# uzh-rpg/EvDeblurNeRF

Hardware: AMD Instinct MI355X
Metric: rays/sec (4096x128 samples, 8x256 MLP) (higher is better)
Workload: dtype f16c (compensated f16: one f16 MFMA product + two block-scaled fp6 MFMA products of the operands' rounding residuals; f32 accumulate; ~2^-15 operands); 1 GPU; nerf8x256 render: 4096 rays x 128 samples per GPU, PE(10,4)+MLP+composite, ndc, viewdirs; rays_per_gpu=4096, samples=128, precision=f16c

## Files before the change

### evdeblurnerf_amd/_lib.py

```python
from __future__ import annotations

import ctypes as C
import os

_HERE = os.path.dirname(os.path.abspath(__file__))
LIB_PATH = os.environ.get("EVD_LIB_PATH") or os.path.join(_HERE, "lib", "libevdnerf.so")
MAXL = 16

PREC = {"f32": 0, "f16x3": 1, "bf16": 2, "f16": 3, "f16c": 4, "f16m": 5}
ACT = {"none": 0, "relu": 1, "sigmoid": 2, "exp": 3, "sigmoid1": 4, "softplus": 5, "tanh": 6}

_fp = C.POINTER(C.c_float)
_vp = C.c_void_p


class EvdError(RuntimeError):
    pass


class RenderCfg(C.Structure):
    _fields_ = [("H", C.c_int), ("W", C.c_int), ("focal", C.c_float),
                ("ndc", C.c_int), ("use_viewdirs", C.c_int), ("lindisp", C.c_int), ("N_samples", C.c_int),
                ("N_importance", C.c_int), ("white_bkgd", C.c_int),
                ("near", C.c_float), ("far", C.c_float), ("perturb", C.c_float),
                ("is_train", C.c_int), ("precision", C.c_int)]


class NerfDesc(C.Structure):
    _fields_ = [("D", C.c_int), ("W", C.c_int), ("multires", C.c_int), ("multires_views", C.c_int), ("skip", C.c_int),
                ("rgb_act", C.c_int), ("sigma_act", C.c_int), ("rmnear", C.c_float),
                ("pts_w", _fp * MAXL), ("pts_b", _fp * MAXL),
                ("views_w", _fp), ("views_b", _fp), ("feature_w", _fp), ("feature_b", _fp),
                ("alpha_w", _fp), ("alpha_b", _fp), ("rgb_w", _fp), ("rgb_b", _fp),
                ("output_w", _fp), ("output_b", _fp), ("output_ch", C.c_int)]


class NerfGrads(C.Structure):
    _fields_ = [("pts_w", _vp * MAXL), ("pts_b", _vp * MAXL),
                ("views_w", _vp), ("views_b", _vp), ("feature_w", _vp), ("feature_b", _vp),
                ("alpha_w", _vp), ("alpha_b", _vp), ("rgb_w", _vp), ("rgb_b", _vp), ("accumulate", C.c_int)]


class VoxelGrads(C.Structure):
    _fields_ = [("sigma_w", _vp * 2), ("color_w", _vp * 3), ("color_b", _vp * 3), ("accumulate", C.c_int)]


class AwpEmbedGrads(C.Structure):
    _fields_ = [("w", _vp * 4), ("b", _vp * 4)]


class AwpTailDesc(C.Structure):
    _fields_ = [("P", C.c_int), ("S", C.c_int), ("VF", C.c_int), ("dir_freqs", C.c_int), ("n_mot", C.c_int), ("training", C.c_int),
                ("bn_eps", C.c_float), ("bn_momentum", C.c_float)]


class VoxelGridGrads(C.Structure):
    _fields_ = [("plane", _vp * 3), ("line", _vp * 3), ("basis", _vp)]


class VoxelDesc(C.Structure):
    _fields_ = [("num_layers", C.c_int), ("hidden_dim", C.c_int), ("geo_feat_dim", C.c_int),
                ("num_layers_color", C.c_int), ("input_ch", C.c_int), ("multires", C.c_int), ("multires_views", C.c_int),
                ("app_dim", C.c_int), ("n_comp", C.c_int * 3), ("grid", C.c_int * 3), ("app_act", C.c_int),
                ("rgb_act", C.c_int), ("sigma_act", C.c_int), ("composite_feature", C.c_int),
                ("aabb", C.c_float * 6), ("rmnear", C.c_float),
                ("sigma_w", _fp * MAXL), ("color_w", _fp * MAXL), ("color_b", _fp * MAXL),
                ("plane", _fp * 3), ("line", _fp * 3), ("basis", _fp)]


class CrfDesc(C.Structure):
    _fields_ = [("map_type", C.c_int), ("gamma", C.c_float), ("extra_features", C.c_int),
                ("w", _fp * 4), ("b", _fp * 4)]


class PoseTrack(C.Structure):
    _fields_ = [("n_keys", C.c_int), ("key_t", _vp), ("key_quat", _vp), ("key_rotvec", _vp), ("trans_coef", _vp),
                ("bd_scale", C.c_float), ("recenter", C.c_int), ("recenter_inv", C.c_double * 12)]


class RigidBlurDesc(C.Structure):
    _fields_ = [(k, C.c_int) for k in ("C", "W_r", "W_v", "W_w", "D_r", "D_v", "D_w", "M", "use_origin", "n_img")] + [("rv_window", C.c_float)]


class RigidBlurParams(C.Structure):
    _fields_ = [(k, _vp) for k in ("table", "r_branch_w", "r_branch_b", "v_branch_w", "v_branch_b", "w_branch_w", "w_branch_b",
                                   "r_linear_w", "r_linear_b", "v_linear_w", "v_linear_b", "w_linear_w", "w_linear_b")]


class LpipsDesc(C.Structure):
    _fields_ = [("conv_w", _fp * 5), ("conv_b", _fp * 5), ("lin", _fp * 5), ("shift", C.c_float * 3), ("scale", C.c_float * 3)]


class RenderOut(C.Structure):
    _fields_ = [(k, _vp) for k in ("rgb", "depth", "acc", "z_vals", "weights", "rgb0", "depth0", "acc0", "z_std",
                                   "z_vals0", "weights0", "feature", "raw")] + [("feature_kind", C.c_int)]


_L, _I, _F, _S = C.c_long, C.c_int, C.c_float, C.c_size_t
SIGNATURES = {
    "evd_last_error": (C.c_char_p, []),
    "evd_version": (_I, []),
    "evd_debug_side_spin_count": (_L, []),
    "evd_compute_successor_workspace_bytes": (_S, [_L]),
    "evd_compute_successor": (_I, [_vp, _L, _L, _vp, _vp, _vp, _vp, _vp, _S, _vp]),
    "evd_event_coord_ids_workspace_bytes": (_S, [_L, _I, _I]),
    "evd_event_coord_ids": (_I, [_vp, _vp, _L, _I, _I, _vp, _vp, _vp, _vp, _vp, _S, _vp]),
    "evd_event_filter_workspace_bytes": (_S, [_L]),
    "evd_event_filter": (_I, [_vp, _vp, _vp, _L, C.c_double, C.c_double, _vp, _vp, _vp, _vp, _S, _vp]),
    "evd_event_color_map_workspace_bytes": (_S, [_L]),
    "evd_event_color_map": (_I, [_vp, _L, _I, _I, _vp, _vp, _vp, _L, _vp, _vp, _vp, _S, _vp]),
    "evd_sample_events": (_I, [_vp, _L, _I, _vp, _L, _vp, _vp, _vp, _vp, _L, _fp, _I, _vp, _vp, _vp, _vp, _vp, _vp, _vp, _vp, _vp]),
    "evd_sample_events_track": (_I, [_vp, _L, _I, _vp, _L, _vp, C.POINTER(PoseTrack), _vp, _vp, _L, _fp, _I, _vp, _vp, _vp, _vp, _vp, _vp, _vp, _vp, _vp]),
    "evd_interpolate_poses": (_I, [C.POINTER(PoseTrack), _vp, _L, _vp, _vp]),
    "evd_image_batch": (_I, [_vp, _L, _vp, _vp, _vp, _I, _I, _I, _fp, _vp, _vp, _vp, _vp, _vp, _vp, _vp, _vp, _vp]),
    "evd_rbk_warp": (_I, [_vp, _vp, _vp, _L, _I, _I, _vp, _vp, _vp]),
    "evd_rigid_blur_workspace_bytes": (_S, [C.POINTER(RigidBlurDesc), _L]),
    "evd_rigid_blur_forward": (_I, [C.POINTER(RigidBlurDesc), C.POINTER(RigidBlurParams), _vp, _vp, _vp, _L, _vp, _vp, _vp, _vp]),
    "evd_rigid_blur_backward": (_I, [C.POINTER(RigidBlurDesc), C.POINTER(RigidBlurParams), _vp, _vp, _vp, _L, _vp, _vp, _vp, _vp, _vp, _vp,
                                     _vp, _S, _vp]),
    "evd_awp_feature_integration": (_I, [_vp, _vp, _vp, _L, _I, _I, _vp, _vp]),
    "evd_awp_feature_integration_bwd": (_I, [_vp, _vp, _vp, _vp, _L, _I, _I, _vp, _vp, _vp, _vp]),
    "evd_mam_local_forward": (_I, [_vp, _vp, _L, _I, _I, _I, _vp, _vp, _vp, _vp, _vp]),
    "evd_mam_local_backward": (_I, [_vp, _vp, _vp, _vp, _vp, _vp, _vp, _vp, _L, _I, _I, _I, _vp, _vp, _I, _vp, _vp]),
    "evd_awp_tail_num_params": (_I, [_I]),
    "evd_awp_tail_param_count": (_L, [C.POINTER(AwpTailDesc)]),
    "evd_awp_tail_workspace_bytes": (_S, [C.POINTER(AwpTailDesc), _L, _I]),
    "evd_awp_tail_saved_floats": (_L, [C.POINTER(AwpTailDesc)]),
    "evd_awp_tail_forward": (_I, [C.POINTER(AwpTailDesc), C.POINTER(_vp), _vp, _vp, _vp, _vp, _vp, _L, _vp, _vp, _vp, _vp, _vp, _vp, _vp, _vp, _vp, _S, _vp]),
    "evd_awp_tail_backward": (_I, [C.POINTER(AwpTailDesc), C.POINTER(_vp), _vp, _vp, _vp, _vp, _vp, _L, _vp, _vp, _vp, _vp, _vp, _vp, _vp, _vp, _vp,
                                   _vp, _vp, _vp, _S, _vp]),
    "evd_awp_local_consumers_backward": (_I, [_vp] * 11 + [_L, _I, _I, _I, _vp, _vp, _vp, _vp, _vp, _vp]),
    "evd_awp_embed_create": (_I, [C.POINTER(_fp), C.POINTER(_fp), _I, _I, _I, C.POINTER(_vp)]),
    "evd_awp_embed_destroy": (None, [_vp]),
    "evd_awp_embed_param_count": (_L, [_vp]),
    "evd_awp_embed_load_params": (_I, [_vp, _vp, _vp]),
    "evd_awp_embed_store_bytes": (_S, [_vp, _L]),
    "evd_awp_embed_backward_workspace_bytes": (_S, []),
    "evd_awp_embed_forward": (_I, [_vp, _I, _vp, _vp, _vp, _S, _L, _vp, _vp, _S, _vp]),
    "evd_awp_embed_backward": (_I, [_vp, _I, _vp, _L, _vp, _S, C.POINTER(AwpEmbedGrads), _vp, _vp, _vp, _S, _vp]),
    "evd_probe_mfma_rate": (_I, [_I, _I, C.POINTER(C.c_double), _vp]),
    "evd_device_count": (_I, []),
    "evd_get_rays": (_I, [_I, _I, _fp, _fp, _I, _vp, _vp, _vp]),
    "evd_get_rays_pix": (_I, [_vp, _fp, _vp, _L, _I, _vp, _vp, _vp]),
    "evd_ndc_rays": (_I, [_I, _I, _F, _F, _vp, _vp, _L, _vp, _vp, _vp]),
    "evd_embed": (_I, [_vp, _L, _I, _I, _vp, _vp]),
    "evd_ray_batch": (_I, [C.POINTER(RenderCfg), _vp, _L, _vp, _vp]),
    "evd_ray_batch_bwd": (_I, [C.POINTER(RenderCfg), _vp, _vp, _L, _vp, _vp]),
    "evd_points": (_I, [_vp, _I, _vp, _L, _I, _vp, _vp]),
    "evd_points_bwd": (_I, [_vp, _vp, _L, _I, _I, _vp, _vp]),
    "evd_sample_z": (_I, [C.POINTER(RenderCfg), _vp, _I, _L, _vp, _vp, _vp]),
    "evd_sample_z_pts": (_I, [C.POINTER(RenderCfg), _vp, _I, _L, _vp, _vp, _vp, _vp]),
    "evd_ray_batch_z": (_I, [C.POINTER(RenderCfg), _vp, _L, _vp, _vp, _vp, _vp]),
    "evd_nerf_create": (_I, [C.POINTER(NerfDesc), C.POINTER(_vp)]),
    "evd_nerf_destroy": (None, [_vp]),
    "evd_nerf_param_count": (_L, [_vp]),
    "evd_nerf_param_blocks": (_I, [_vp, C.POINTER(C.c_long), _I]),
    "evd_nerf_load_params": (_I, [_vp, _vp, _vp]),
    "evd_nerf_stream_bytes": (_S, [_vp, _I]),
    "evd_nerf_mlp": (_I, [_vp, _I, _vp, _vp, _L, _I, _vp, _vp, _I, _vp]),
    "evd_nerf_train_store_bytes": (_S, [_L]),
    "evd_nerf_train_store_bytes_prec": (_S, [_I, _L]),
    "evd_nerf_mlp_train": (_I, [_vp, _I, _vp, _vp, _L, _I, _vp, _vp, _S, _vp]),
    "evd_nerf_backward_workspace_bytes": (_S, []),
    "evd_nerf_mlp_backward": (_I, [_vp, _I, _vp, _L, _I, _vp, _S, C.POINTER(NerfGrads), _vp, _vp, _I, _vp, _vp, _vp, _S, _vp]),
    "evd_voxel_param_count": (_L, [_vp]),
    "evd_voxel_param_blocks": (_I, [_vp, C.POINTER(C.c_long), _I]),
    "evd_voxel_load_params": (_I, [_vp, _vp, _vp]),
    "evd_voxel_train_store_bytes": (_S, [_vp, _L]),
    "evd_voxel_train_store_bytes_prec": (_S, [_vp, _I, _L]),
    "evd_voxel_backward_workspace_bytes": (_S, []),
    "evd_voxel_mlp_train": (_I, [_vp, _I, _vp, _vp, _I, _vp, _I, _L, _I, _vp, _vp, _vp, _S, _vp]),
    "evd_voxel_geo_feat_dim": (_I, [_vp]),
    "evd_voxel_mlp_backward": (_I, [_vp, _I, _vp, _vp, _vp, _vp, _S, _L, _I, _vp, _S, C.POINTER(VoxelGrads), _vp, _I, _vp, _vp, _I, _vp, _vp, _vp, _S, _vp]),
    "evd_voxel_grid_sizes": (_I, [_vp, C.POINTER(C.c_long)]),
    "evd_voxel_get_grids": (_I, [_vp, C.POINTER(_vp), C.POINTER(_vp), _vp, _vp]),
    "evd_voxel_load_grids": (_I, [_vp, C.POINTER(_vp), C.POINTER(_vp), _vp, _vp]),
    "evd_voxel_sample_bwd": (_I, [_vp, _vp, _L, _vp, _I, _I, C.POINTER(VoxelGridGrads), _vp, _vp]),
    "evd_voxel_sample_bwd_workspace_bytes": (_S, [_vp, _L]),
    "evd_voxel_sample_bwd_ws": (_I, [_vp, _vp, _L, _vp, _I, _I, C.POINTER(VoxelGridGrads), _vp, _vp, _S, _vp]),
    "evd_voxel_sample_bwd_prec": (_I, [_vp, _I, _vp, _L, _vp, _I, _I, C.POINTER(VoxelGridGrads), _vp, _vp, _S, _vp]),
    "evd_voxel_tv_loss_bwd": (_I, [_vp, _vp, C.POINTER(VoxelGridGrads), _vp]),
    "evd_raw2outputs": (_I, [_vp, _vp, _vp, _I, _L, _I, _I, _I, _I, _I, _I, _I, _I, _F, _vp,
                             _vp, _vp, _vp, _vp, _vp, _vp, _I, _vp, _vp]),
    "evd_raw2outputs_bwd": (_I, [_vp, _vp, _vp, _I, _L, _I, _I, _I, _I, _I, _I, _I, _I, _F, _vp, _vp, _vp, _vp, _vp, _vp, _vp]),
    "evd_raw2outputs_bwd_rays": (_I, [_vp, _vp, _vp, _I, _L, _I, _I, _I, _I, _I, _I, _I, _I, _F, _vp, _vp, _vp, _vp, _vp, _vp, _vp, _I, _vp]),
    "evd_sample_pdf_merge": (_I, [_vp, _vp, _L, _I, _I, _I, _vp, _vp, _vp, _vp, _vp, _vp]),
    "evd_nerf_render_workspace_bytes": (_S, [C.POINTER(RenderCfg), _L]),
    "evd_nerf_render_rays": (_I, [_vp, _vp, C.POINTER(RenderCfg), _vp, _L, _vp, _vp, _vp, _vp,
                                  C.POINTER(RenderOut), _vp, _S, _vp]),
    "evd_nerf_render": (_I, [_vp, _vp, C.POINTER(RenderCfg), _vp, _L, _vp, _vp, _vp, _vp,
                             C.POINTER(RenderOut), _vp, _S, _vp]),
    "evd_voxel_create": (_I, [C.POINTER(VoxelDesc), C.POINTER(_vp)]),
    "evd_voxel_destroy": (None, [_vp]),
    "evd_voxel_sample": (_I, [_vp, _vp, _L, _vp, _I, _I, _vp]),
    "evd_voxel_sample_prec": (_I, [_vp, _I, _vp, _L, _vp, _I, _I, _vp]),
    "evd_voxel_forward": (_I, [_vp, _I, _vp, _vp, _I, _vp, _I, _vp, _vp, _I, _L, _I, _I,
                               _vp, _vp, _vp, _vp, _vp, _vp, _S, _vp]),
    "evd_voxel_forward_workspace_bytes": (_S, [_vp, _L, _I]),
    "evd_c2f_render_workspace_bytes": (_S, [_vp, _vp, C.POINTER(RenderCfg), _L]),
    "evd_c2f_render_rays": (_I, [_vp, _vp, C.POINTER(RenderCfg), _vp, _L, _vp, _vp, _vp, _vp,
                                 C.POINTER(RenderOut), _vp, _S, _vp]),
    "evd_c2f_render": (_I, [_vp, _vp, C.POINTER(RenderCfg), _vp, _L, _vp, _vp, _vp, _vp,
                            C.POINTER(RenderOut), _vp, _S, _vp]),
    "evd_voxel_tv_loss": (_I, [_vp, _vp, _vp]),
    "evd_merge_features": (_I, [_vp, _vp, _vp, _L, _I, _I, _I, _vp, _I, _vp]),
    "evd_merge_features_bwd": (_I, [_vp, _I, _vp, _L, _I, _I, _I, _vp, _vp, _vp]),
    "evd_weighted_sum": (_I, [_vp, _vp, _L, _I, _I, _vp, _vp]),
    "evd_crf_create": (_I, [C.POINTER(CrfDesc), C.POINTER(_vp)]),
    "evd_crf_destroy": (None, [_vp]),
    "evd_crf_forward": (_I, [_vp, _vp, _vp, _I, _I, _I, _L, _vp, _vp]),
    "evd_blur_loss_reduce": (_I, [_vp, _I, _vp, _vp, _vp, _vp, _vp, _vp, _L, _I, _vp, _vp, _vp, _vp, _vp]),
    "evd_crf_param_count": (_I, []),
    "evd_crf_get_params": (_I, [_vp, _vp]),
    "evd_crf_load_params": (_I, [_vp, _vp]),
    "evd_event_loss_bwd": (_I, [_vp, _I, _I, _I, _vp, _vp, _vp, _vp, _vp, _vp, _F, _F, _vp, _fp, _L, _F, _F, _vp, _vp, _vp, _vp, _vp, _vp]),
    "evd_blur_loss_bwd": (_I, [_vp, _I, _vp, _vp, _vp, _vp, _vp, _vp, _L, _I, _fp, _vp, _vp, _vp, _vp, _vp]),
    "evd_blur_loss_bwd_dev": (_I, [_vp, _I, _vp, _vp, _vp, _vp, _vp, _vp, _L, _I, _vp, _vp, _vp, _vp, _vp, _vp]),
    "evd_event_loss_bwd_dev": (_I, [_vp, _I, _I, _I, _vp, _vp, _vp, _vp, _vp, _vp, _F, _F, _vp, _fp, _L, _vp, _vp, _vp, _vp, _vp, _vp, _vp]),
    "evd_event_loss_reduce": (_I, [_vp, _I, _I, _I, _vp, _vp, _vp, _vp, _vp, _vp, _F, _F, _vp, _fp, _L, _vp, _vp]),
    "evd_numerics_flags": (_I, [C.POINTER(_vp), C.POINTER(C.c_long), _I, _vp, _vp]),
    "evd_edi_deblur": (_I, [_vp, _vp, _I, _L, _vp, _vp]),
    "evd_edi_bii_image": (_I, [_vp, _vp, _vp, _L, _I, _I, _F, _F, _vp, _vp]),
    "evd_edi_prior_workspace_bytes": (_S, [_I, _I, _I, _I]),
    "evd_edi_prior": (_I, [_vp, _L, _vp, _L, _vp, _vp, _I, _I, _I, _I, _F, _F, _vp, _vp, _vp, _vp, _S, _vp]),
    "evd_img_metrics_workspace_bytes": (_S, [_I, _I, _I]),
    "evd_img_metrics": (_I, [_vp, _vp, _vp, _I, _I, _I, _I, _I, _I, _vp, _vp, _S, _vp]),
    "evd_to8b": (_I, [_vp, _L, _vp, _vp]),
    "evd_lpips_create": (_I, [C.POINTER(LpipsDesc), C.POINTER(_vp)]),
    "evd_lpips_destroy": (None, [_vp]),
    "evd_lpips_workspace_bytes": (_S, [_I, _I, _I]),
    "evd_lpips": (_I, [_vp, _vp, _vp, _I, _I, _I, _vp, _vp, _S, _vp]),
}

_lib = None


def _share_torch_hip_runtime():
    import torch
    tl = os.path.join(os.path.dirname(torch.__file__), "lib", "libamdhip64.so")
    if os.path.exists(tl):
        C.CDLL(tl, mode=C.RTLD_GLOBAL)


def lib():
    global _lib
    if _lib is None:
        if not os.path.exists(LIB_PATH):
            raise EvdError(f"{LIB_PATH} not found: build it with `python -m evdeblurnerf_amd.build` "
                           "(hipcc, --offload-arch=gfx950). There is no CPU fallback.")
        _share_torch_hip_runtime()
        handle = C.CDLL(LIB_PATH)
        for name, (res, args) in SIGNATURES.items():
            fn = getattr(handle, name)
            fn.restype = res
            fn.argtypes = args
        _lib = handle
    return _lib


def check(rc: int, what: str = ""):
    if rc != 0:
        msg = lib().evd_last_error()
        raise EvdError(f"{what or 'libevdnerf'} failed ({rc}): {msg.decode() if msg else '?'}")


def ptr(t):
    if t is None:
        return None
    if not t.is_contiguous():
        raise EvdError("tensor must be contiguous")
    return C.c_void_p(t.data_ptr())


def stream_ptr():
    import torch
    return C.c_void_p(torch.cuda.current_stream().cuda_stream)


_BACKWARD_GEN = [0]


def backward_generation():
    return _BACKWARD_GEN[0]


def note_backward():
    _BACKWARD_GEN[0] += 1
```

### evdeblurnerf_amd/csrc/evd_api.hip

```cpp
#include <atomic>
#include "evd_common.h"
#include "nerf_mlp.h"
#include "nerf_mlp_kernel.h"
#include "nerf_net.h"
#include "nerf_train.h"
#include "pack.h"

#include <cmath>
#include <cstdint>
#include <cstdlib>
#include <cstring>
#include <vector>

namespace evd {

char* err_buf() {
    static thread_local char buf[512] = {0};
    return buf;
}

int fail(int code, const char* fmt, ...) {
    va_list ap;
    va_start(ap, fmt);
    vsnprintf(err_buf(), 512, fmt, ap);
    va_end(ap);
    return code;
}

int nerf_mlp_generic_dispatch(int prec, int W, const MlpParams& p, hipStream_t st);
int nerf_mlp_pipe_dispatch(int prec, const MlpParams& p, hipStream_t st);
int nerf_mlp_c_dispatch(int W, int D, int skip, const MlpParams& p, hipStream_t st);
int nerf_mlp_c_chunks(int W, int D, int skip, bool train);

static __global__ void k_fold_feature(const float* __restrict__ views_w, const float* __restrict__ views_b, const float* __restrict__ feature_w,
                                      const float* __restrict__ feature_b, int W, int ICV, float* __restrict__ wfold, float* __restrict__ bfold) {
    const int in = W + ICV, rows = W / 2;
    const long i = (long)blockIdx.x * 256 + threadIdx.x;
    if (i < (long)rows * in) {
        const int r = (int)(i / in), c = (int)(i % in);
        if (c >= W) { wfold[i] = views_w[i]; return; }
        double acc = 0.0;
        for (int k = 0; k < W; ++k) acc = fma((double)views_w[(long)r * in + k], (double)feature_w[(long)k * W + c], acc);
        wfold[i] = (float)acc;
    } else if (i < (long)rows * in + rows) {
        const int r = (int)(i - (long)rows * in);
        double acc = 0.0;
        for (int k = 0; k < W; ++k) acc = fma((double)views_w[(long)r * in + k], (double)feature_b[k], acc);
        bfold[r] = (float)(acc + (double)views_b[r]);
    }
}

static int nerf_fold_pack(evd_nerf* n, const float* params, hipStream_t st) {
    if (!n->pipe_cf.data.p) return EVD_OK;
    const int W = n->W, D = n->D, ICV = 3 * (1 + 2 * n->multires_views);
    const long total = n->param_off[n->nparam_blocks], nw = (long)(W / 2) * (W + ICV), nel = nw + W / 2;
    float* ext = (float*)n->fold_arena.p;
    EVD_HIP(hipMemcpyAsync(ext, params, (size_t)total * sizeof(float), hipMemcpyDeviceToDevice, st));
    hipLaunchKernelGGL(k_fold_feature, dim3((unsigned)cdiv(nel, 256L)), dim3(256), 0, st, ext + n->param_off[2 * D], ext + n->param_off[2 * D + 1],
                       ext + n->param_off[2 * D + 2], ext + n->param_off[2 * D + 3], W, ICV, ext + total, ext + total + nw);
    EVD_LAUNCH_CHECK();
    int rc = repack_stream_c(n->pipe_cf, ext, st);
    if (rc) return rc;
    const long nb = (long)(n->bias_f.bytes / sizeof(float));
    hipLaunchKernelGGL(k_gather_f32, dim3((unsigned)cdiv(nb, 256L)), dim3(256), 0, st, (const float*)ext, (const int*)n->bias_f_src.p, nb, (float*)n->bias_f.p);
    EVD_LAUNCH_CHECK();
    return EVD_OK;
}

static std::atomic<long> g_side_spins{0};
static __global__ void k_test_spin(long long ticks) {
    const long long t0 = wall_clock64();
    while (wall_clock64() - t0 < ticks) __builtin_amdgcn_s_sleep(32);
}
int test_side_spin(hipStream_t side) {
    static const int us = [] { const char* e = getenv("EVD_TEST_SIDE_SPIN_US"); return e ? atoi(e) : 0; }();
    if (us <= 0) return EVD_OK;
    hipLaunchKernelGGL(k_test_spin, dim3(1), dim3(64), 0, side, (long long)us * 100);
    EVD_LAUNCH_CHECK();
    g_side_spins.fetch_add(1, std::memory_order_relaxed);
    return EVD_OK;
}
bool test_skip_side_join() {
    static const bool skip = [] { const char* e = getenv("EVD_TEST_SKIP_SIDE_JOIN"); return e && e[0] == '1'; }();
    return skip;
}

}

using namespace evd;

extern "C" {

const char* evd_last_error(void) { return evd::err_buf(); }
long evd_debug_side_spin_count(void) { return evd::g_side_spins.load(std::memory_order_relaxed); }
int evd_version(void) { return 120; }

int evd_device_count(void) {
    int n = 0;
    if (hipGetDeviceCount(&n) != hipSuccess) return fail(EVD_E_NODEVICE, "hipGetDeviceCount failed");
    return n;
}

static int upload_stream(evd_nerf::Packed& dst, const StreamBuilder& sb) { return dst.upload(sb); }

static void nerf_param_sizes(int D, int W, int skip, int L, int Lv, long* sz) {
    const int IC = 3 * (1 + 2 * L), ICV = 3 * (1 + 2 * Lv);
    for (int l = 0; l < D; ++l) {
        sz[2 * l] = (long)W * (l == 0 ? IC : (l - 1 == skip ? W + IC : W));
        sz[2 * l + 1] = W;
    }
    long* h = sz + 2 * D;
    h[0] = (long)(W / 2) * (W + ICV); h[1] = W / 2;
    h[2] = (long)W * W; h[3] = W;
    h[4] = W; h[5] = 1;
    h[6] = 3L * (W / 2); h[7] = 3;
}

int evd_nerf_create(const evd_nerf_desc* d, evd_nerf** out) {
    EVD_REQUIRE(d && out, "evd_nerf_create: null argument");
    EVD_REQUIRE(d->multires >= 0 && d->multires <= PE_L_MAX && d->multires_views >= 0 && pe_ksteps(d->multires_views) <= 4,
                "evd_nerf_create: multires %d / multires_views %d out of range (0..%d / 0..10)", d->multires, d->multires_views, PE_L_MAX);
    const int L = d->multires, Lv = d->multires_views, VKS = pe_ksteps(Lv) <= 2 ? 2 : 4;
    const bool standard = L == PE_L && Lv == PE_LV;
    EVD_REQUIRE(d->W == 256 || d->W == 64, "evd_nerf_create: netwidth %d not built (64, 256)", d->W);
    EVD_REQUIRE(d->D >= 1 && d->D <= EVD_MAX_LAYERS, "evd_nerf_create: netdepth %d out of range", d->D);
    const bool no_views = !d->views_w && !d->feature_w && !d->alpha_w && !d->rgb_w && d->output_w;
    EVD_REQUIRE(no_views || (d->views_w && d->feature_w && d->alpha_w && d->rgb_w),
                "evd_nerf_create: give either the view branch (views / feature / alpha / rgb) or output_linear (use_viewdirs=False)");
    EVD_REQUIRE(!no_views || (d->output_b && (d->output_ch == 4 || d->output_ch == 5)), "evd_nerf_create: output_linear needs its bias and output_ch 4 or 5");
    const int W = d->W, T = W / 32, KS = W / 16, IC = 3 * (1 + 2 * L), ICV = 3 * (1 + 2 * Lv), D = d->D;
    evd_nerf* n = new evd_nerf();
    n->multires = L; n->multires_views = Lv;
    n->D = D; n->W = W; n->skip = d->skip; n->rgb_act = d->rgb_act; n->sigma_act = d->sigma_act; n->rmnear = d->rmnear;
    n->no_views = no_views ? 1 : 0;

    long sz[2 * EVD_MAX_LAYERS + 8];
    nerf_param_sizes(D, W, d->skip, L, Lv, sz);
    n->nparam_blocks = 2 * D + 8;
    if (no_views) {
        sz[2 * D] = (long)d->output_ch * W; sz[2 * D + 1] = d->output_ch;
        n->nparam_blocks = 2 * D + 2;
    }
    long total = 0;
    for (int i = 0; i < n->nparam_blocks; ++i) { n->param_off[i] = total; total += sz[i]; }
    n->param_off[n->nparam_blocks] = total;
    std::vector<float> arena((size_t)total, 0.f);
    {
        const float* srcs[2 * EVD_MAX_LAYERS + 8];
        for (int l = 0; l < D; ++l) { srcs[2 * l] = d->pts_w[l]; srcs[2 * l + 1] = d->pts_b[l]; }
        const float* heads[8] = {d->views_w, d->views_b, d->feature_w, d->feature_b, d->alpha_w, d->alpha_b, d->rgb_w, d->rgb_b};
        for (int i = 0; i < 8; ++i) srcs[2 * D + i] = heads[i];
        if (no_views) { srcs[2 * D] = d->output_w; srcs[2 * D + 1] = d->output_b; }
        for (int i = 0; i < n->nparam_blocks; ++i)
            if (srcs[i]) memcpy(arena.data() + n->param_off[i], srcs[i], sz[i] * sizeof(float));
    }
    const float* A = arena.data();
    auto P = [&](int i) { return A + n->param_off[i]; };
    auto pts_w = [&](int l) { return P(2 * l); };
    const float *views_w = P(2 * D), *feature_w = no_views ? nullptr : P(2 * D + 2), *alpha_w = no_views ? nullptr : P(2 * D + 4), *rgb_w = no_views ? nullptr : P(2 * D + 6);
    const float* output_w = P(2 * D);
    const int out_rows = d->output_ch < 4 ? d->output_ch : 4;

    auto pe_col = [L](int j, int kk) { return pe_src_col(L, 8 * j + (kk & 7), kk >> 3); };
    auto hid_col = [](int j, int kk) { return 16 * j + phi(kk); };
    auto views_col = [&](int j, int kk) {
        if (j < KS) return hid_col(j, kk);
        const int c = pe_src_col(Lv, 8 * (j - KS) + (kk & 7), kk >> 3);
        return c < 0 ? -1 : W + c;
    };
    auto build = [&](StreamBuilder& sb, int pdh) {
        sb.layer(pts_w(0), W, IC, T, PE_KS, true, pe_col);
        for (int l = 1; l < D; ++l) {
            if (l - 1 == d->skip) {
                auto wide_col = [&](int j, int kk) {
                    if (pdh < 0) return j < PE_KS ? pe_col(j, kk) : IC + hid_col(j - PE_KS, kk);
                    if (j < pdh) return IC + hid_col(j, kk);
                    if (j < pdh + PE_KS) return pe_col(j - pdh, kk);
                    return IC + hid_col(j - PE_KS, kk);
                };
                sb.layer(pts_w(l), W, W + IC, T, PE_KS + KS, true, wide_col);
            } else {
                sb.layer(pts_w(l), W, W, T, KS, true, hid_col);
            }
        }
        if (no_views) {
            sb.layer(output_w, out_rows, W, 1, KS, true, hid_col);
            return;
        }
        sb.layer(alpha_w, 1, W, 1, KS, false, hid_col);
        sb.layer(feature_w, W, W, T, KS, false, hid_col);
        sb.layer(views_w, W / 2, W + ICV, T / 2, KS + VKS, false, views_col);
        sb.layer(rgb_w, 3, W / 2, 1, KS / 2, true, hid_col);
    };
    int rc = EVD_OK;
    for (int prec = 0; prec < EVD_NUM_PREC && !rc; ++prec) {
        if (prec == EVD_PREC_F16C) {
            n->nchunks[prec] = n->pipe_chunks[prec] = 0;
            if (no_views || !standard || !nerf_mlp_c_chunks(W, D, d->skip, false)) continue;
            auto build_c = [&](StreamBuilderC& sc, const float* base, bool fold) {
                auto Pb = [&](int i) { return base + n->param_off[i]; };
                sc.arena = base;
                const int KB = KS / 4;
                sc.layer(Pb(0), W, IC, T, PE_KS, 2, pe_col);
                for (int l = 1; l < D; ++l) {
                    if (l - 1 == d->skip) {
                        auto wide_col = [&](int j, int kk) {
                            if (j < 4 * (KB - 1)) return IC + c_hid_col(j, kk);
                            if (j < 4 * (KB - 1) + PE_KS) return pe_col(j - 4 * (KB - 1), kk);
                            return IC + c_hid_col(j - PE_KS, kk);
                        };
                        sc.layer(Pb(2 * l), W, W + IC, T, PE_KS + KS, 2, wide_col);
                    } else {
                        sc.layer(Pb(2 * l), W, W, T, KS, 2, c_hid_col);
                    }
                }
                sc.layer(Pb(2 * D + 4), 1, W, 1, KS, 1, c_hid_col);
                if (!fold) sc.layer(Pb(2 * D + 2), W, W, T, KS, 2, c_hid_col);
                sc.layer(fold ? base + total : Pb(2 * D), W / 2, W + ICV, T / 2, KS + PEV_KS, 2, [&](int j, int kk) {
                    if (j < KS) return c_hid_col(j, kk);
                    const int c = pe_src_col(Lv, 8 * (j - KS) + (kk & 7), kk >> 3);
                    return c < 0 ? -1 : W + c;
                });
                sc.layer(Pb(2 * D + 6), 3, W / 2, 1, KS / 2, 1, c_hid_col);
            };
            StreamBuilderC sc(PIPE_CB);
            build_c(sc, A, false);
            n->pipe_chunks[prec] = (int)(sc.bytes.size() / PIPE_CB);
            if (n->pipe_chunks[prec] != nerf_mlp_c_chunks(W, D, d->skip, true)) rc = fail(EVD_E_INVALID, "evd_nerf_create: f16c stream has %d chunks, kernel expects %d", n->pipe_chunks[prec], nerf_mlp_c_chunks(W, D, d->skip, true));
            if (!rc) rc = n->pipe_c.upload(sc);
            if (rc) continue;
            const long nfold = (long)(W / 2) * (W + ICV) + W / 2;
            std::vector<float> ext((size_t)(total + nfold), 0.f);
            StreamBuilderC sf(PIPE_CB);
            build_c(sf, ext.data(), true);
            n->fold_chunks = (int)(sf.bytes.size() / PIPE_CB);
            if (n->fold_chunks != nerf_mlp_c_chunks(W, D, d->skip, false)) rc = fail(EVD_E_INVALID, "evd_nerf_create: folded f16c stream has %d chunks, kernel expects %d", n->fold_chunks, nerf_mlp_c_chunks(W, D, d->skip, false));
            if (!rc) rc = n->pipe_cf.upload(sf);
            if (!rc) rc = n->fold_arena.alloc(ext.size() * sizeof(float));
            continue;
        }
        StreamBuilder sb(prec);
        sb.arena = A;
        build(sb, -1);
        n->nchunks[prec] = (int)(sb.bytes.size() / chunk_bytes(prec));
        rc = upload_stream(n->stream[prec], sb);
        n->pipe_chunks[prec] = 0;
        if (!rc && !no_views && standard && nerf_pipe_built(prec, W, D, d->skip)) {
            StreamBuilder sp(prec, PIPE_CB);
            sp.arena = A;
            sp.group = nerf_group(prec);
            build(sp, KS - 2 * nerf_group(prec));
            n->pipe_chunks[prec] = (int)(sp.bytes.size() / PIPE_CB);
            rc = upload_stream(n->pipe[prec], sp);
        }
        if (rc || !is_train_prec(prec) || !n->pipe_chunks[prec]) continue;
        auto put = [&](int which, auto fill) {
            StreamBuilder sb2(prec, PIPE_CB);
            sb2.arena = A;
            sb2.group = 1;
            fill(sb2);
            return upload_stream(n->bwd[prec][which], sb2);
        };
        rc = put(EVD_BWD_RGB, [&](StreamBuilder& b) { b.layer_transposed(rgb_w, 3, W / 2, 0, W / 2, nullptr, 0, T / 2, 1, true, [](int, int kk) { return kk < 3 ? kk : -1; }); });
        if (!rc) rc = put(EVD_BWD_VIEWS, [&](StreamBuilder& b) { b.layer_transposed(views_w, W / 2, W + ICV, 0, W, nullptr, 0, T, KS / 2, true, hid_col); });
        if (!rc) rc = put(EVD_BWD_HEAD, [&](StreamBuilder& b) {
            b.layer_transposed(feature_w, W, W, 0, W, alpha_w, 1, T, KS + 1, true, [&](int j, int kk) { return j < KS ? hid_col(j, kk) : (kk == 0 ? W : -1); });
        });
        auto enc_row = [](int L_, int idx) { const int j = idx / 16, kk = phi_inv(idx % 16); return pe_src_col(L_, 8 * j + (kk & 7), kk >> 3); };
        auto enc_layer = [&](StreamBuilder& b, const float* Wm, int in_dim, int col0, int L_, int tiles, int ksteps) {
            b.layer_at(tiles, ksteps, true, [&](int t, int r) { const int c = enc_row(L_, 32 * t + r); return c < 0 ? -1 : col0 + c; }, hid_col,
                       [=](int r, int c) { return Wm + (size_t)c * in_dim + r; });
        };
        if (!rc) rc = put(EVD_BWD_PE0, [&](StreamBuilder& b) { enc_layer(b, pts_w(0), IC, 0, PE_L, 2, KS); });
        if (!rc && d->skip >= 0 && d->skip + 1 < D) rc = put(EVD_BWD_PESKIP, [&](StreamBuilder& b) { enc_layer(b, pts_w(d->skip + 1), W + IC, 0, PE_L, 2, KS); });
        if (!rc) rc = put(EVD_BWD_DIR, [&](StreamBuilder& b) { enc_layer(b, views_w, W + ICV, W, PE_LV, 1, KS / 2); });
        for (int l = 1; l < D && !rc; ++l) {
            const bool wide = l - 1 == d->skip;
            rc = put(EVD_BWD_HIDDEN1 + l - 1, [&](StreamBuilder& b) { b.layer_transposed(pts_w(l), W, wide ? W + IC : W, wide ? IC : 0, W, nullptr, 0, T, KS, true, hid_col); });
        }
    }
    if (rc) { evd_nerf_destroy(n); return rc; }
    {
        std::vector<int> m(MAP_TOTAL, -1);
        for (int i = 0; i < 256; ++i) {
            m[MAP_HID + i] = hid_col(i / 16, i % 16);
            m[MAP_HID_SKIP + i] = IC + hid_col(i / 16, i % 16);
        }
        for (int i = 0; i < 64; ++i) m[MAP_PE + i] = pe_col(i / 16, i % 16);
        for (int i = 0; i < 32; ++i) {
            const int c = pe_src_col(Lv, 8 * (i / 16) + (i % 16 & 7), (i % 16) >> 3);
            m[MAP_DIR + i] = c < 0 ? -1 : W + c;
        }
        for (int i = 0; i < 3; ++i) m[MAP_RGB + i] = i;
        m[MAP_ALPHA] = 0;
        if ((rc = n->wmaps.upload(m.data(), m.size() * sizeof(int)))) { evd_nerf_destroy(n); return rc; }
    }
    std::vector<float> b;
    std::vector<int32_t> bsrc;
    auto push = [&](int block, int out_dim, int tiles) {
        for (int i = 0; i < tiles * 32; ++i) {
            b.push_back(i < out_dim ? P(block)[i] : 0.f);
            bsrc.push_back(i < out_dim ? (int32_t)(n->param_off[block] + i) : -1);
        }
    };
    for (int l = 0; l < D; ++l) push(2 * l + 1, W, T);
    if (no_views) {
        push(2 * D + 1, out_rows, 1);
    } else {
        push(2 * D + 5, 1, 1);
        push(2 * D + 3, W, T);
        push(2 * D + 1, W / 2, T / 2);
        push(2 * D + 7, 3, 1);
    }
    rc = n->bias.upload(b.data(), b.size() * sizeof(float));
    if (!rc) rc = n->bias_src.upload(bsrc.data(), bsrc.size() * sizeof(int32_t));
    if (!rc && n->pipe_cf.data.p) {
        const long nw = (long)(W / 2) * (W + ICV);
        std::vector<int32_t> fsrc(bsrc.begin(), bsrc.begin() + (D * T + 1) * 32);
        for (int i = 0; i < (T / 2) * 32; ++i) fsrc.push_back((int32_t)(total + nw + i));
        fsrc.insert(fsrc.end(), bsrc.end() - 32, bsrc.end());
        rc = n->bias_f_src.upload(fsrc.data(), fsrc.size() * sizeof(int32_t));
        if (!rc) rc = n->bias_f.alloc(fsrc.size() * sizeof(float));
        DevBuf dev_params;
        if (!rc) rc = dev_params.upload(arena.data(), arena.size() * sizeof(float));
        if (!rc) rc = nerf_fold_pack(n, (const float*)dev_params.p, nullptr);
        if (!rc && hipStreamSynchronize(nullptr) != hipSuccess) rc = fail(EVD_E_HIP, "evd_nerf_create: the folded f16c stream could not be packed");
        dev_params.release();
    }
    if (rc) { evd_nerf_destroy(n); return rc; }
    *out = n;
    return EVD_OK;
}

void evd_nerf_destroy(evd_nerf* n) {
    if (!n) return;
    for (int i = 0; i < EVD_NUM_PREC; ++i) {
        n->stream[i].release();
        n->pipe[i].release();
        for (int k = 0; k < EVD_BWD_NSTREAMS; ++k) n->bwd[i][k].release();
    }
    n->wmaps.release();
    n->batch.release();
    n->bias.release();
    n->bias_src.release();
    n->pipe_c.release();
    n->pipe_cf.release();
    n->bias_f.release();
    n->bias_f_src.release();
    n->fold_arena.release();
    n->side.release();
    delete n;
}

long evd_nerf_param_count(const evd_nerf* net) { return net ? net->param_off[net->nparam_blocks] : 0; }

int evd_nerf_param_blocks(const evd_nerf* net, long* offsets, int capacity) {
    EVD_REQUIRE(net, "evd_nerf_param_blocks: null network");
    if (offsets)
        for (int i = 0; i <= net->nparam_blocks && i < capacity; ++i) offsets[i] = net->param_off[i];
    return net->nparam_blocks;
}

int evd_nerf_load_params(evd_nerf* net, const float* params, void* stream) {
    EVD_REQUIRE(net && params, "evd_nerf_load_params: null argument");
    hipStream_t st = as_stream(stream);
    int rc;
    std::vector<PackedStream*> all;
    for (int i = 0; i < EVD_NUM_PREC; ++i) {
        all.push_back(&net->stream[i]);
        all.push_back(&net->pipe[i]);
        for (int k = 0; k < EVD_BWD_NSTREAMS; ++k) all.push_back(&net->bwd[i][k]);
    }
    if ((rc = repack_batch(net->batch, all, params, st))) return rc;
    if ((rc = repack_stream_c(net->pipe_c, params, st))) return rc;
    const long nb = (long)(net->bias.bytes / sizeof(float));
    hipLaunchKernelGGL(k_gather_f32, dim3((unsigned)cdiv(nb, 256L)), dim3(256), 0, st, params, (const int*)net->bias_src.p, nb, (float*)net->bias.p);
    EVD_LAUNCH_CHECK();
    return nerf_fold_pack(net, params, st);
}

size_t evd_nerf_stream_bytes(const evd_nerf* net, int precision) {
    if (!net || precision < 0 || precision >= EVD_NUM_PREC) return 0;
    if (precision == EVD_PREC_F16C) return net->pipe_cf.data.bytes;
    return net->pipe_chunks[precision] ? net->pipe[precision].data.bytes : net->stream[precision].data.bytes;
}

int evd_nerf_mlp(const evd_nerf* net, int precision, const float* ray_batch, const float* z, long R, int S,
                 float* raw, float* feature, int feature_kind, void* stream) {
    EVD_REQUIRE(net && ray_batch && z && raw, "evd_nerf_mlp: null argument");
    EVD_REQUIRE(precision >= 0 && precision < EVD_NUM_PREC, "evd_nerf_mlp: unknown precision %d", precision);
    EVD_REQUIRE(R >= 0 && S >= 1, "evd_nerf_mlp: bad shape R=%ld S=%d", R, S);
    EVD_REQUIRE(!feature || feature_kind == 1 || feature_kind == 2, "evd_nerf_mlp: feature_kind must be 1 or 2");
    if (R == 0) return EVD_OK;
    MlpParams p{};
    const bool piped = net->pipe_chunks[precision] > 0;
    p.wstream = (const char*)(piped ? net->pipe[precision].data.p : net->stream[precision].data.p);
    p.bias = (const float*)net->bias.p;
    p.ray_batch = ray_batch; p.z = z; p.nsamp = R * (long)S; p.S = S; p.ncol = net->no_views ? 8 : 11; p.no_views = net->no_views;
    p.pe_l = net->multires; p.pe_lv = net->multires_views;
    EVD_REQUIRE(!(net->no_views && feature && feature_kind == 1), "evd_nerf_mlp: a use_viewdirs=False network has no after_linear feature (nerf.py:159)");
    EVD_REQUIRE(!net->no_views || precision != EVD_PREC_F16C, "evd_nerf_mlp: EVD_PREC_F16C is not built for use_viewdirs=False networks");
    p.D = net->D; p.skip = net->skip; p.nchunks = piped ? net->pipe_chunks[precision] : net->nchunks[precision]; p.nbias = (int)(net->bias.bytes / sizeof(float));
    p.raw = raw; p.feature = feature; p.feature_kind = feature ? feature_kind : 0; p.act = nullptr; p.wscale = nullptr;
    if (precision == EVD_PREC_F16C) {
        EVD_REQUIRE(net->pipe_chunks[precision] > 0, "evd_nerf_mlp: EVD_PREC_F16C is built for netdepth 8, netwidth 256, skips [4], multires 10 / 4 only");
        EVD_REQUIRE(!feature, "evd_nerf_mlp: EVD_PREC_F16C has no feature-row variant (use EVD_PREC_F16X3)");
        p.wstream = (const char*)net->pipe_cf.data.p;
        p.nchunks = net->fold_chunks;
        p.wscale = (const unsigned*)net->pipe_cf.scales.p;
        p.bias = (const float*)net->bias_f.p;
        p.nbias = (int)(net->bias_f.bytes / sizeof(float));
        return nerf_mlp_c_dispatch(net->W, net->D, net->skip, p, as_stream(stream));
    }
    if (piped) return nerf_mlp_pipe_dispatch(precision, p, as_stream(stream));
    return nerf_mlp_generic_dispatch(precision, net->W, p, as_stream(stream));
}

static size_t align256(size_t x) { return (x + 255) & ~(size_t)255; }

size_t evd_nerf_render_workspace_bytes(const evd_render_cfg* cfg, long R) {
    if (!cfg || R < 0) return 0;
    const size_t S = cfg->N_samples, Ni = cfg->N_importance > 0 ? cfg->N_importance : 0, St = S + Ni, r = (size_t)R;
    size_t b = 0;
    b += align256(r * 11 * 4);
    b += align256(r * St * 4);
    b += align256(r * S * 4);
    b += align256(r * St * 16);
    b += align256(r * St * 4);
    b += align256(r * S * 4);
    b += align256(r * (Ni ? Ni : 1) * 4);
    return b + 256;
}

}
static float* render_z_slot(const evd_render_cfg* cfg, long R, const evd_render_out* out, void* workspace) {
    const int S = cfg->N_samples, Ni = cfg->N_importance > 0 ? cfg->N_importance : 0, St = S + Ni;
    char* w = (char*)(((uintptr_t)workspace + 255) & ~(uintptr_t)255);
    w += align256((size_t)R * 11 * 4) + align256((size_t)R * St * 4);
    float* z0 = (float*)w;
    return Ni ? (out->z_vals0 ? out->z_vals0 : z0) : (out->z_vals ? out->z_vals : z0);
}
static int render_rays_impl(const evd_nerf* coarse, const evd_nerf* fine, const evd_render_cfg* cfg, const float* rb,
                            long R, const float* t_rand, const float* u, const float* noise0, const float* noise1,
                            evd_render_out* out, void* workspace, size_t workspace_bytes, void* stream, bool z_done) {
    EVD_REQUIRE(coarse && cfg && out && (rb || R == 0), "evd_nerf_render_rays: null argument");
    EVD_REQUIRE((cfg->use_viewdirs != 0) == (coarse->no_views == 0) && (!fine || fine->no_views == coarse->no_views),
                "evd_nerf_render_rays: cfg->use_viewdirs does not match the networks (view branch vs output_linear)");
    const int nc = cfg->use_viewdirs ? 11 : 8;
    EVD_REQUIRE(cfg->N_samples >= 1, "evd_nerf_render_rays: N_samples must be >= 1");
    EVD_REQUIRE(cfg->N_importance <= 0 || fine, "evd_nerf_render_rays: N_importance > 0 needs the fine network");
    EVD_REQUIRE(cfg->N_importance <= 0 || cfg->N_samples >= 3, "evd_nerf_render_rays: hierarchical sampling needs N_samples >= 3");
    EVD_REQUIRE(!(cfg->perturb > 0.f) || (t_rand && (cfg->N_importance <= 0 || u)),
                "evd_nerf_render_rays: perturb > 0 needs explicit t_rand (and u) draws");
    if (R == 0) return EVD_OK;
    const size_t need = evd_nerf_render_workspace_bytes(cfg, R);
    if (!workspace || workspace_bytes < need)
        return fail(EVD_E_WORKSPACE, "evd_nerf_render_rays: workspace %zu < %zu bytes", workspace_bytes, need);
    const int S = cfg->N_samples, Ni = cfg->N_importance > 0 ? cfg->N_importance : 0, St = S + Ni;
    char* w = (char*)(((uintptr_t)workspace + 255) & ~(uintptr_t)255);
    auto take = [&](size_t bytes) { char* p = w; w += align256(bytes); return (float*)p; };
    const size_t r = (size_t)R;
    (void)take(r * 11 * 4);
    float* z2 = take(r * St * 4);
    float* z0 = take(r * S * 4);
    float* raw = take(r * St * 16);
    float* wts = take(r * St * 4);
    float* wts0 = take(r * S * 4);
    float* zs = take(r * (Ni ? Ni : 1) * 4);
    int rc;
    float* zc = (Ni ? (out->z_vals0 ? out->z_vals0 : z0) : (out->z_vals ? out->z_vals : z0));
    if (!z_done && (rc = evd_sample_z(cfg, rb, nc, R, t_rand, zc, stream))) return rc;
    auto pass = [&](const evd_nerf* net, const float* z, int Sp, const float* noise, float* rgb, float* depth, float* acc,
                    float* weights, float* raw_out, float* feat) -> int {
        int rc2 = evd_nerf_mlp(net, cfg->precision, rb, z, R, Sp, raw_out, feat, out->feature_kind ? out->feature_kind : 1, stream);
        if (rc2) return rc2;
        const float thr = (!cfg->is_train && net->rmnear > 0.f) ? (float)((double)net->rmnear / 128.0) : 0.f;
        return evd_raw2outputs(raw_out, z, rb + 3, nc, R, Sp, 4, 3, 0, 3, net->rgb_act, net->sigma_act, cfg->white_bkgd, thr,
                               noise, rgb, nullptr, acc, weights, depth, nullptr, 0, nullptr, stream);
    };
    if (!Ni) {
        float* wo = out->weights ? out->weights : wts;
        float* ro = out->raw ? out->raw : raw;
        return pass(coarse, zc, S, noise0, out->rgb, out->depth, out->acc, wo, ro, out->feature);
    }
    float* w0 = out->weights0 ? out->weights0 : wts0;
    if ((rc = pass(coarse, zc, S, noise0, out->rgb0, out->depth0, out->acc0, w0, raw, nullptr))) return rc;
    float* zm = out->z_vals ? out->z_vals : z2;
    if ((rc = evd_sample_pdf_merge(zc, w0, R, S, Ni, cfg->perturb == 0.f, u, zs, zm, nullptr, out->z_std, stream))) return rc;
    float* wo = out->weights ? out->weights : wts;
    float* ro = out->raw ? out->raw : raw;
    return pass(fine, zm, St, noise1, out->rgb, out->depth, out->acc, wo, ro, out->feature);
}

extern "C" {
int evd_nerf_render_rays(const evd_nerf* coarse, const evd_nerf* fine, const evd_render_cfg* cfg, const float* rb,
                         long R, const float* t_rand, const float* u, const float* noise0, const float* noise1,
                         evd_render_out* out, void* workspace, size_t workspace_bytes, void* stream) {
    return render_rays_impl(coarse, fine, cfg, rb, R, t_rand, u, noise0, noise1, out, workspace, workspace_bytes, stream, false);
}

int evd_nerf_render(const evd_nerf* coarse, const evd_nerf* fine, const evd_render_cfg* cfg, const float* rays, long R,
                    const float* t_rand, const float* u, const float* noise0, const float* noise1,
                    evd_render_out* out, void* workspace, size_t workspace_bytes, void* stream) {
    EVD_REQUIRE(cfg && out && (rays || R == 0), "evd_nerf_render: null argument");
    if (R == 0) return EVD_OK;
    const size_t need = evd_nerf_render_workspace_bytes(cfg, R);
    if (!workspace || workspace_bytes < need)
        return fail(EVD_E_WORKSPACE, "evd_nerf_render: workspace %zu < %zu bytes", workspace_bytes, need);
    float* rb = (float*)(((uintptr_t)workspace + 255) & ~(uintptr_t)255);
    const bool fused_z = cfg->use_viewdirs && cfg->N_samples >= 1;
    int rc = fused_z ? evd_ray_batch_z(cfg, rays, R, t_rand, rb, render_z_slot(cfg, R, out, workspace), stream) : evd_ray_batch(cfg, rays, R, rb, stream);
    if (rc) return rc;
    return render_rays_impl(coarse, fine, cfg, rb, R, t_rand, u, noise0, noise1, out, workspace, workspace_bytes, stream, fused_z);
}

}
```

### evdeblurnerf_amd/csrc/kernel_nerf_mlp_pipe_f16c.hip

```cpp
#include "nerf_mlp_c_kernel.h"

namespace evd {

int nerf_mlp_c_chunks(int W, int D, int skip, bool train) {
    if (!nerf_c_built(W, D, skip)) return 0;
    return train ? nerf_c_chunks<256, 8, 4, true>() : nerf_c_chunks<256, 8, 4, false>();
}

int nerf_mlp_c_dispatch(int W, int D, int skip, const MlpParams& p, hipStream_t st) {
    if (nerf_c_built(W, D, skip)) return launch_nerf_c<256, 8, 4>(p, st);
    return fail(EVD_E_INVALID, "evd_nerf_mlp: EVD_PREC_F16C is built for netdepth 8, netwidth 256, skips [4] only");
}

}
```

### evdeblurnerf_amd/csrc/mlp_pipe_c.h

```cpp
#pragma once

#include <cstdlib>

#include "mlp_pipe.h"

namespace evd {

typedef const __attribute__((address_space(3))) float* lds_f32_p;
typedef const __attribute__((address_space(3))) f32x4* lds_f32x4_p;
typedef const __attribute__((address_space(3))) unsigned* lds_u32_p;

typedef int i32x8 __attribute__((ext_vector_type(8)));
typedef int i32x6 __attribute__((ext_vector_type(6)));
typedef unsigned u32x4 __attribute__((ext_vector_type(4)));
typedef unsigned u32x2 __attribute__((ext_vector_type(2)));
typedef unsigned u32x16 __attribute__((ext_vector_type(16)));
typedef _Float16 f16x32 __attribute__((ext_vector_type(32)));

struct CCfg {
    static constexpr int NT = 256, NW = 4, CB = PIPE_CB, FB = 1024, UPC = CB / 1024, PIECES = CB / 1024 / NW;
    static constexpr int NSLOT = 4;
    static constexpr int BARP = 1;
    static constexpr int PDM = 4;
    static constexpr int SAMPLES = NW * 32;
    static constexpr int RING = NSLOT * CB;
    static constexpr int BIAS_WORDS = 5120;
    static constexpr int TOTAL = RING + BIAS_WORDS * 4;
    static_assert((NSLOT & (NSLOT - 1)) == 0 && NSLOT >= 4 && NSLOT - BARP >= BARP + 1 && NSLOT - BARP >= 3 && TOTAL <= 160 * 1024, "ring geometry");
};

static inline int c_persistent_blocks() {
    static const int n = [] {
        int dev = 0, cus = 0;
        if (hipGetDevice(&dev) != hipSuccess || hipDeviceGetAttribute(&cus, hipDeviceAttributeMultiprocessorCount, dev) != hipSuccess || cus <= 0) cus = 256;
        return cus;
    }();
    return n;
}
static inline long cmin_l(long a, long b) { return a < b ? a : b; }

template <int NCH> struct CStream {
    static constexpr int kChunks = NCH, NSLOT = CCfg::NSLOT, BARP = CCfg::BARP;
    static constexpr int AHEAD = NSLOT - BARP;
    const char* gbase;
    const char* rd_base;
    unsigned voff;
    unsigned dst0;
    static_assert(CCfg::PIECES == 4, "four 1 KiB pieces per wavefront per chunk");
    __device__ __forceinline__ void issue(int c) {
        const unsigned off = voff + (unsigned)c * CCfg::CB;
        const unsigned dst = dst0 + (unsigned)(c & (NSLOT - 1)) * CCfg::CB;
        asm volatile("s_mov_b32 m0, %2\n\ts_nop 0\n\t"
                     "global_load_lds_dwordx4 %0, %1\n\tglobal_load_lds_dwordx4 %0, %1 offset:1024\n\t"
                     "global_load_lds_dwordx4 %0, %1 offset:2048\n\tglobal_load_lds_dwordx4 %0, %1 offset:3072"
                     : : "v"(off), "s"(gbase), "s"(dst) : "memory");
    }
    __device__ __forceinline__ void issue_piece(int c, int k) {
        const unsigned off = voff + (unsigned)c * CCfg::CB;
        const unsigned dst_next = dst0 + (unsigned)((c + 1) & (NSLOT - 1)) * CCfg::CB;
        if (k == 0) asm volatile("global_load_lds_dwordx4 %0, %1" : : "v"(off), "s"(gbase) : "memory");
        else if (k == 1) asm volatile("global_load_lds_dwordx4 %0, %1 offset:1024" : : "v"(off), "s"(gbase) : "memory");
        else if (k == 2) asm volatile("global_load_lds_dwordx4 %0, %1 offset:2048" : : "v"(off), "s"(gbase) : "memory");
        else asm volatile("global_load_lds_dwordx4 %0, %1 offset:3072\n\ts_mov_b32 m0, %2" : : "v"(off), "s"(gbase), "s"(dst_next) : "memory");
    }
    __device__ __forceinline__ void set_m0_for(int c) {
        const unsigned dst = dst0 + (unsigned)(c & (NSLOT - 1)) * CCfg::CB;
        asm volatile("s_mov_b32 m0, %0" : : "s"(dst) : "memory");
    }
    static __device__ __forceinline__ void wait_chunks(int chunks) {
        switch (chunks) {
        case 0: wait_vmcnt<0>(); break;
        case 1: wait_vmcnt<4>(); break;
        case 2: wait_vmcnt<8>(); break;
        case 3: wait_vmcnt<12>(); break;
        case 4: wait_vmcnt<16>(); break;
        case 5: wait_vmcnt<20>(); break;
        case 6: wait_vmcnt<24>(); break;
        default: wait_vmcnt<28>(); break;
        }
    }
    __device__ __forceinline__ void start_issue(const char* g, char* ring, int tid) {
        const int wave = __builtin_amdgcn_readfirstlane(tid >> 6), lane = tid & 63;
        gbase = g;
        voff = wave * (CCfg::PIECES * 1024) + lane * 16;
        rd_base = ring + lane * 16;
        dst0 = __builtin_amdgcn_readfirstlane(lds_offset_of(ring) + wave * (CCfg::PIECES * 1024));
#pragma unroll
        for (int c = 0; c < AHEAD; ++c)
            if (c < NCH) issue(c);
        set_m0_for(AHEAD);
    }
    __device__ __forceinline__ void restart_issue() {
#pragma unroll
        for (int c = 0; c < AHEAD; ++c)
            if (c < NCH) issue(c);
        set_m0_for(AHEAD);
    }
    __device__ __forceinline__ void start_wait() {
        wait_chunks(cmax(0, cmin(AHEAD, NCH) - (BARP + 1)));
        __syncthreads();
    }
    __device__ __forceinline__ void chunk_end(int c) {
        if ((c + 1) % BARP != 0) return;
        wait_chunks(cmax(0, cmin(c + AHEAD, NCH - 1) - (c + BARP + 1)));
        __builtin_amdgcn_s_barrier();
        asm volatile("" ::: "memory");
    }
};

struct XBlk {
    u32x16 h;
    i32x8 qh, ql;
    unsigned sc;
};

__device__ __forceinline__ f16x8 xblk_frag(const XBlk& x, int jj) {
    u32x4 w;
    w[0] = x.h[4 * jj]; w[1] = x.h[4 * jj + 1]; w[2] = x.h[4 * jj + 2]; w[3] = x.h[4 * jj + 3];
    return __builtin_bit_cast(f16x8, w);
}

template <bool SIGNED> __device__ __forceinline__ unsigned c_max_acc(unsigned m, unsigned w) {
    typedef unsigned short u16x2 __attribute__((ext_vector_type(2)));
    if (SIGNED) w &= 0x7fff7fffu;
    return __builtin_bit_cast(unsigned, __builtin_elementwise_max(__builtin_bit_cast(u16x2, m), __builtin_bit_cast(u16x2, w)));
}

__device__ __forceinline__ unsigned c_scales(unsigned m) {
    const unsigned ma = m & 0xffffu, mb = m >> 16;
    const unsigned mm = ma > mb ? ma : mb;
    const unsigned e16 = (mm >> 10) & 31u;
    const unsigned bh = e16 + 110u;
#ifdef EVD_C_RNE
    return bh | ((bh - 11u) << 8);
#else
    return bh | ((bh - 10u) << 8);
#endif
}

__device__ __forceinline__ void c_finish(XBlk& x, unsigned m, const f32x16& r0, const f32x16& r1) {
    const unsigned sc = c_scales(m);
    x.sc = sc;
    const float sh = __builtin_bit_cast(float, (sc & 255u) << 23), sl = __builtin_bit_cast(float, ((sc >> 8) & 255u) << 23);
    i32x6 qh, ql;
    asm("v_cvt_scalef32_pk32_fp6_f16 %0, %1, %2" : "=&v"(qh) : "v"(x.h), "v"(sh));
    asm("v_cvt_scalef32_2xpk16_fp6_f32 %0, %1, %2, %3" : "=&v"(ql) : "v"(r0), "v"(r1), "v"(sl));
#pragma unroll
    for (int e = 0; e < 6; ++e) { x.qh[e] = qh[e]; x.ql[e] = ql[e]; }
    x.qh[6] = x.qh[7] = x.ql[6] = x.ql[7] = 0;
}

template <bool RELU>
__device__ __forceinline__ void c_drain_pair(f32x16& a0, f32x16& a1, int v, XBlk& x, unsigned& m) {
    float x0 = a0[v], x1 = a1[v];
#ifdef EVD_C_RNE
    if (RELU) { x0 = relu_f32(x0); x1 = relu_f32(x1); }
    const f32x2 xv = {x0, x1};
    const unsigned w = __builtin_bit_cast(unsigned, __builtin_convertvector(xv, f16x2));
    constexpr bool CLAMP = false;
#else
    unsigned w = __builtin_bit_cast(unsigned, __builtin_amdgcn_cvt_pkrtz(x0, x1));
    if (RELU) {
        const s16x2 zero = {0, 0};
        const unsigned wraw = w;
        w = __builtin_bit_cast(unsigned, __builtin_elementwise_max(__builtin_bit_cast(s16x2, wraw), zero));
        m = __builtin_bit_cast(unsigned, __builtin_elementwise_max(__builtin_bit_cast(s16x2, m), __builtin_bit_cast(s16x2, wraw)));
    }
    constexpr bool CLAMP = RELU;
#endif
    x.h[v] = w;
#ifdef EVD_C_RNE
    m = c_max_acc<!RELU>(m, w);
#else
    if (!RELU) m = c_max_acc<true>(m, w);
#endif
    float r0, r1;
    if (CLAMP) {
        asm("v_fma_mix_f32 %0, %1, -1.0, %2 op_sel_hi:[1,0,0] clamp" : "=v"(r0) : "v"(w), "v"(x0));
        asm("v_fma_mix_f32 %0, %1, -1.0, %2 op_sel:[1,0,0] op_sel_hi:[1,0,0] clamp" : "=v"(r1) : "v"(w), "v"(x1));
    } else {
        asm("v_fma_mix_f32 %0, %1, -1.0, %2 op_sel_hi:[1,0,0]" : "=v"(r0) : "v"(w), "v"(x0));
        asm("v_fma_mix_f32 %0, %1, -1.0, %2 op_sel:[1,0,0] op_sel_hi:[1,0,0]" : "=v"(r1) : "v"(w), "v"(x1));
    }
    a0[v] = r0;
    a1[v] = r1;
}

template <int NBLK_, int LASTK_, int TILES_, int G_, bool RELU_, bool F32OUT_, int CHUNK0_, int PAR_, int PG_, bool PRELU_, int PDB_, int NEXT_G_,
          int OSLOT_ = -1, int PSLOT_ = -1, int MSLOT_ = -1, int PMSLOT_ = -1, int PFRAG0_ = -1>
struct CLayer {
    static constexpr int NBLK = NBLK_, LASTK = LASTK_, TILES = TILES_, G = G_, CHUNK0 = CHUNK0_, PAR = PAR_, PG = PG_, PDB = PDB_, NEXT_G = NEXT_G_;
    static constexpr int OSLOT = OSLOT_, PSLOT = PSLOT_, MSLOT = MSLOT_, PMSLOT = PMSLOT_;
    static constexpr int PFRAG0 = PFRAG0_ >= 0 ? PFRAG0_ : 4 * PDB_;
    static constexpr bool RELU = RELU_, F32OUT = F32OUT_, PRELU = PRELU_;
    static constexpr int NG = TILES_ / G_;
    static constexpr int KSTEPS = 4 * (NBLK_ - 1) + LASTK_;
    static constexpr int nk(int b) { return b == NBLK_ - 1 ? LASTK_ : 4; }
    static constexpr int blk_units(int b) { return nk(b) * G_ + 3 * G_; }
    static constexpr int blk_slots(int b) { return nk(b) * G_ + 2 * G_; }
    static constexpr int GROUP_UNITS = (NBLK_ - 1) * (4 * G_ + 3 * G_) + LASTK_ * G_ + 3 * G_;
    static constexpr int GROUP_SLOTS = (NBLK_ - 1) * (4 * G_ + 2 * G_) + LASTK_ * G_ + 2 * G_;
    static constexpr int UNITS = NG * GROUP_UNITS;
    static constexpr int NCHUNKS = cceil(UNITS, CCfg::UPC);
    static constexpr int PAR_OUT = (PAR_ + NG) & 1;
    static constexpr int main_pos(int p, int mi) { return p * GROUP_UNITS + (mi / (4 * G_)) * 7 * G_ + mi % (4 * G_); }
    static constexpr int NMAIN = KSTEPS * TILES_;
    static_assert(TILES_ % G_ == 0 && (G_ == 1 || G_ == 2), "groups of one or two tiles");
    static_assert(NMAIN % CCfg::PDM == 0, "the float16 fragment ring keeps its phase across layers");
    static_assert(UNITS % CCfg::UPC == 0 || UNITS % CCfg::UPC >= 2, "a layer's last chunk must reach its second unit");
};

struct CPipe {
    f16x8 am[CCfg::PDM];
    i32x8 ac[2][2];
    f32x16 acc[2][2];
    unsigned wsc[2][2];
    unsigned m;
    unsigned mbits[4];
};

struct CAct {
    const char* base;
    unsigned voff;
};
__device__ __forceinline__ void c_act_store(const CAct& a, int slot, const u32x4& v) {
    const char* sb = a.base + (long)(slot >> 2) * 4096;
    switch (slot & 3) {
    case 0: asm volatile("global_store_dwordx4 %0, %1, %2" EVD_ACT_NT_ASM "\n\ts_nop 1" : : "v"(a.voff), "v"(v), "s"(sb) : "memory"); break;
    case 1: asm volatile("global_store_dwordx4 %0, %1, %2 offset:1024" EVD_ACT_NT_ASM "\n\ts_nop 1" : : "v"(a.voff), "v"(v), "s"(sb) : "memory"); break;
    case 2: asm volatile("global_store_dwordx4 %0, %1, %2 offset:2048" EVD_ACT_NT_ASM "\n\ts_nop 1" : : "v"(a.voff), "v"(v), "s"(sb) : "memory"); break;
    default: asm volatile("global_store_dwordx4 %0, %1, %2 offset:3072" EVD_ACT_NT_ASM "\n\ts_nop 1" : : "v"(a.voff), "v"(v), "s"(sb) : "memory"); break;
    }
}

template <bool MASK>
__device__ __forceinline__ void c_store_block(const CAct& act, int slot, const XBlk& x, unsigned (&mbits)[4], int fi0) {
#pragma unroll
    for (int tt = 0; tt < 2; ++tt) {
#pragma unroll
        for (int f = 0; f < 2; ++f) {
            unsigned w[4];
#pragma unroll
            for (int e = 0; e < 4; ++e) w[e] = __builtin_amdgcn_perm(x.h[8 * f + 2 * e + 1], x.h[8 * f + 2 * e], tt ? 0x07060302u : 0x05040100u);
            const int fo = 2 * tt + f;
            const u32x4 v = {w[0], w[1], w[2], w[3]};
            c_act_store(act, slot + fo, v);
            if (MASK) mbits[(fi0 + fo) >> 2] |= bits_of_words(w) << (8 * ((fi0 + fo) & 3));
        }
    }
}
template <int NK> __device__ __forceinline__ void c_store_input(const CAct& act, int slot, const XBlk& x) {
#pragma unroll
    for (int jj = 0; jj < NK; ++jj) {
        const u32x4 v = {x.h[4 * jj], x.h[4 * jj + 1], x.h[4 * jj + 2], x.h[4 * jj + 3]};
        c_act_store(act, slot + jj, v);
    }
}

template <class L> __device__ __forceinline__ constexpr int c_ring_off(int u) { return ((L::CHUNK0 + u / CCfg::UPC) & (CCfg::NSLOT - 1)) * CCfg::CB + (u % CCfg::UPC) * 1024; }

template <class L, class NXT, class ST, int NIN, int NOUT, int P, bool TRAIN = false>
__device__ __forceinline__ void c_group(ST& st, CPipe& pp, XBlk (&in)[NIN], XBlk (&out)[NOUT], lds_f32_p bias, int lane, const CAct& act = CAct{}) {
    constexpr int G = L::G, NS = L::GROUP_SLOTS;
    constexpr int cur = (L::PAR + P) & 1, oth = cur ^ 1;
    constexpr bool FIRST = P == 0, LAST = P == L::NG - 1;
    constexpr int DG = FIRST ? L::PG : G;
    constexpr int QU = DG > 0 ? DG * 8 + 1 : 0;
    constexpr int NBL0 = (P == L::NG - 1 ? L::NEXT_G : G) * 5;
    constexpr int s_dep = (FIRST && L::PG > 0) ? L::PDB * (4 * G + 2 * G) : NS;
    constexpr int dend = cmin(s_dep, NS - cceil(NBL0, 3) - 1);
    constexpr bool drain_first = QU > 0 && dend - 2 < 1;
    constexpr int drate = (QU > 0 && !drain_first) ? cceil(QU, dend - 2) : (drain_first ? QU : 0);
    constexpr int BG = LAST ? L::NEXT_G : G;
    constexpr int NBL = BG * 5;
    constexpr int b0 = cmin(drain_first ? 0 : dend - 1, NS - 1);
    constexpr int brate = NBL > 0 ? cceil(NBL, NS - b0) : 0;
    auto units_thru = [](int s) constexpr { return (QU == 0 || s < 0) ? 0 : (drain_first ? QU : (s < 2 ? 0 : cmin(QU, ((s - 1) * QU) / (dend - 2)))); };
    auto bias_thru = [](int s) constexpr { return (NBL == 0 || s <= b0) ? 0 : (s >= NS ? NBL : cmin(NBL, (s - b0) * brate)); };
    const int h = lane >> 5;
    lds_f32_p bias_next = bias + (LAST ? L::TILES : (P + 1) * G) * 32;
    constexpr int SC_OFF = CCfg::BIAS_WORDS / 2;
    constexpr int ubase = P * L::GROUP_UNITS;
    constexpr int mbase = P * L::KSTEPS * G;

    auto filler = [&](int s) __attribute__((always_inline)) {
#pragma unroll
        for (int i = 0; i < drate; ++i) {
            const int u = units_thru(s - 1) + i;
            if (u < units_thru(s)) {
                XBlk& dst = FIRST ? in[L::PDB] : out[P > 0 ? P - 1 : 0];
                if (u < DG * 8) {
                    static_assert(DG == 0 || DG == 2, "blocks are drained from groups of two tiles");
                    if (u == 0) pp.m = 0u;
                    if (FIRST) c_drain_pair<L::PRELU>(pp.acc[oth][0], pp.acc[oth][1], u, dst, pp.m);
                    else c_drain_pair<L::RELU>(pp.acc[oth][0], pp.acc[oth][1], u, dst, pp.m);
                } else {
                    c_finish(dst, pp.m, pp.acc[oth][0], pp.acc[oth][1]);
                    if constexpr (TRAIN) {
                        if constexpr (FIRST) {
                            if constexpr (L::PSLOT >= 0) {
                                c_store_block<(L::PMSLOT >= 0)>(act, L::PSLOT, dst, pp.mbits, L::PFRAG0);
                                if constexpr (L::PMSLOT >= 0) {
                                    const u32x4 mv = {pp.mbits[0], pp.mbits[1], pp.mbits[2], pp.mbits[3]};
                                    c_act_store(act, L::PMSLOT, mv);
                                    pp.mbits[0] = pp.mbits[1] = pp.mbits[2] = pp.mbits[3] = 0u;
                                }
                            }
                        } else if constexpr (L::OSLOT >= 0) {
                            c_store_block<(L::MSLOT >= 0)>(act, L::OSLOT + 4 * (P > 0 ? P - 1 : 0), dst, pp.mbits, 4 * (P > 0 ? P - 1 : 0));
                        }
                    }
                }
            }
        }
#pragma unroll
        for (int i = 0; i < brate; ++i) {
            const int b = bias_thru(s - 1) + i;
            if (b < bias_thru(s)) {
                const int bt = b / 5, q = b % 5;
                if (q < 4) {
                    const f32x4 bv = *(lds_f32x4_p)(bias_next + bt * 32 + 8 * q + 4 * h);
#pragma unroll
                    for (int e = 0; e < 4; ++e) pp.acc[oth][bt][4 * q + e] = bv[e];
                } else {
                    pp.wsc[oth][bt] = ((lds_u32_p)bias_next)[SC_OFF + bt * 32 + (lane & 31)];
                }
            }
        }
    };
    auto chunks = [&](int t0, int t1) __attribute__((always_inline)) {
        const int c0 = t0 / CCfg::UPC, c1 = t1 / CCfg::UPC;
        auto due = [](int t) constexpr { return cmin(CCfg::PIECES, (t + 1) / 3); };
        auto pieces = [&](int c, int k0, int k1) __attribute__((always_inline)) {
            if (c + ST::AHEAD >= ST::kChunks) return;
#pragma unroll
            for (int k = 0; k < CCfg::PIECES; ++k)
                if (k >= k0 && k < k1) st.issue_piece(c + ST::AHEAD, k);
        };
        if (c0 == c1) {
            pieces(L::CHUNK0 + c0, due(t0 % CCfg::UPC), due(t1 % CCfg::UPC));
        } else {
            pieces(L::CHUNK0 + c0, due(t0 % CCfg::UPC), CCfg::PIECES);
            st.chunk_end(L::CHUNK0 + c0);
            pieces(L::CHUNK0 + c1, 0, due(t1 % CCfg::UPC));
        }
    };

    int s = 0, ub = ubase, mm = mbase;
#pragma unroll
    for (int b = 0; b < L::NBLK; ++b) {
        const int nk = L::nk(b);
        const int lo16 = ub + nk * G, hi8 = lo16 + 2 * G;
        const int ncl = 4 * G;
        const int per_slot = cceil(ncl, nk * G);
#pragma unroll
        for (int jj = 0; jj < nk; ++jj) {
#pragma unroll
            for (int t = 0; t < G; ++t) {
                const int i = jj * G + t;
                filler(s);
                {
                    constexpr int LA = CCfg::PDM - 1;
                    const int idx = mm + LA - mbase;
                    int u = -1, ringoff = 0;
                    if (idx < L::KSTEPS * G) {
                        u = L::main_pos(P, idx);
                        ringoff = c_ring_off<L>(u);
                    } else if (!LAST) {
                        u = L::main_pos(P + 1, idx - L::KSTEPS * G);
                        ringoff = c_ring_off<L>(u);
                    } else if constexpr (!std::is_void<NXT>::value) {
                        if ((ub + i) / CCfg::UPC >= L::NCHUNKS - 1) {
                            u = NXT::main_pos(0, idx - L::KSTEPS * G);
                            ringoff = c_ring_off<NXT>(u);
                        }
                    }
                    if (u >= 0) pp.am[(mm + LA) % CCfg::PDM] = *reinterpret_cast<const f16x8*>(st.rd_base + ringoff);
                }
#pragma unroll
                for (int q = 0; q < per_slot; ++q) {
                    const int c = i * per_slot + q;
                    if (c < ncl) {
                        const int kt = c >> 1, part = c & 1;
                        const int kind = kt / G, tt = kt % G;
                        if (part == 0) {
                            const u32x4 w = *reinterpret_cast<const u32x4*>(st.rd_base + c_ring_off<L>(lo16 + kt));
#pragma unroll
                            for (int e = 0; e < 4; ++e) pp.ac[kind][tt][e] = (int)w[e];
                        } else {
                            const int uo = hi8 + kt / 2;
                            const u32x2 w = *reinterpret_cast<const u32x2*>(st.rd_base + c_ring_off<L>(uo) - 8 * lane + (kt & 1) * 512);
                            pp.ac[kind][tt][4] = (int)w[0];
                            pp.ac[kind][tt][5] = (int)w[1];
                            pp.ac[kind][tt][6] = 0;
                            pp.ac[kind][tt][7] = 0;
                        }
                    }
                }
                __builtin_amdgcn_sched_barrier(0);
                pp.acc[cur][t] = __builtin_amdgcn_mfma_f32_32x32x16_f16(pp.am[mm % CCfg::PDM], xblk_frag(in[b], jj), pp.acc[cur][t], 0, 0, 0);
                __builtin_amdgcn_sched_barrier(0);
                chunks(ub + i, ub + i + 1);
                ++s;
                ++mm;
            }
        }
#pragma unroll
        for (int kind = 0; kind < 2; ++kind) {
#pragma unroll
            for (int t = 0; t < G; ++t) {
                const int i = kind * G + t;
                filler(s);
                __builtin_amdgcn_sched_barrier(0);
                int sca = (int)pp.wsc[cur][t], scb = (int)in[b].sc;
                if (TRAIN) asm("" : "+v"(sca), "+v"(scb));
                if (kind == 0)
                    pp.acc[cur][t] = __builtin_amdgcn_mfma_scale_f32_32x32x64_f8f6f4(pp.ac[0][t], in[b].qh, pp.acc[cur][t], 2, 2, 0, sca, 0, scb);
                else
                    pp.acc[cur][t] = __builtin_amdgcn_mfma_scale_f32_32x32x64_f8f6f4(pp.ac[1][t], in[b].ql, pp.acc[cur][t], 2, 2, 1, sca, 1, scb);
                __builtin_amdgcn_sched_barrier(0);
                const int last = 2 * G - 1;
                chunks(lo16 + i, i == last ? hi8 + G : lo16 + i + 1);
                ++s;
            }
        }
        ub = hi8 + G;
    }
#pragma unroll
    for (int i = 0; i < NBL; ++i) {
        const int bq = bias_thru(NS - 1) + i;
        if (bq < NBL) {
            const int bt = bq / 5, q = bq % 5;
            if (q < 4) {
                const f32x4 bv = *(lds_f32x4_p)(bias_next + bt * 32 + 8 * q + 4 * h);
#pragma unroll
                for (int e = 0; e < 4; ++e) pp.acc[oth][bt][4 * q + e] = bv[e];
            } else {
                pp.wsc[oth][bt] = ((lds_u32_p)bias_next)[SC_OFF + bt * 32 + (lane & 31)];
            }
        }
    }
}

template <class L, class NXT, class ST, int NIN, int NOUT, int P, bool TRAIN = false> struct CGroupLoop {
    static __device__ __forceinline__ void run(ST& st, CPipe& pp, XBlk (&in)[NIN], XBlk (&out)[NOUT], lds_f32_p bias, int lane, const CAct& act = CAct{}) {
        c_group<L, NXT, ST, NIN, NOUT, P, TRAIN>(st, pp, in, out, bias, lane, act);
        if constexpr (P + 1 < L::NG) CGroupLoop<L, NXT, ST, NIN, NOUT, P + 1, TRAIN>::run(st, pp, in, out, bias, lane, act);
    }
};

template <class L, class NXT, class ST, int NIN, int NOUT, bool TRAIN = false>
__device__ __forceinline__ void c_layer(ST& st, CPipe& pp, XBlk (&in)[NIN], XBlk (&out)[NOUT], float* out_f32, lds_f32_p bias, int lane, const CAct& act = CAct{}) {
    static_assert(NIN >= L::NBLK, "input blocks");
    CGroupLoop<L, NXT, ST, NIN, NOUT, 0, TRAIN>::run(st, pp, in, out, bias, lane, act);
    if (L::UNITS % CCfg::UPC != 0) {
        constexpr int c = L::CHUNK0 + L::UNITS / CCfg::UPC, k0 = cmin(CCfg::PIECES, (L::UNITS % CCfg::UPC + 1) / 3);
        if (c + ST::AHEAD < ST::kChunks) {
#pragma unroll
            for (int k = k0; k < CCfg::PIECES; ++k) st.issue_piece(c + ST::AHEAD, k);
        }
        st.chunk_end(L::CHUNK0 + L::UNITS / CCfg::UPC);
    }
    if constexpr (!std::is_void<NXT>::value) {
#pragma unroll
        for (int k = 0; k < CCfg::PDM - 1; ++k)
            if (L::main_pos(L::NG - 1, L::KSTEPS * L::G - (CCfg::PDM - 1) + k) / CCfg::UPC < L::NCHUNKS - 1)
                pp.am[k] = *reinterpret_cast<const f16x8*>(st.rd_base + c_ring_off<NXT>(NXT::main_pos(0, k)));
    }
    if (L::F32OUT) {
        constexpr int cur = (L::PAR + L::NG - 1) & 1;
#pragma unroll
        for (int r = 0; r < 4; ++r) {
            out_f32[r] = pp.acc[cur][0][r];
            asm volatile("" : "+v"(out_f32[r]));
        }
    }
}

template <class L, class ST> __device__ __forceinline__ void c_prime(ST& st, CPipe& pp, lds_f32_p bias, int lane) {
    const int h = lane >> 5;
#pragma unroll
    for (int i = 0; i < CCfg::PDM - 1; ++i) pp.am[i] = *reinterpret_cast<const f16x8*>(st.rd_base + c_ring_off<L>(L::main_pos(0, i)));
#pragma unroll
    for (int t = 0; t < L::G; ++t) {
#pragma unroll
        for (int q = 0; q < 4; ++q) {
            const f32x4 bv = *(lds_f32x4_p)(bias + t * 32 + 8 * q + 4 * h);
#pragma unroll
            for (int e = 0; e < 4; ++e) pp.acc[L::PAR][t][4 * q + e] = bv[e];
        }
        pp.wsc[L::PAR][t] = ((lds_u32_p)bias)[CCfg::BIAS_WORDS / 2 + t * 32 + (lane & 31)];
    }
    pp.m = 0u;
    pp.mbits[0] = pp.mbits[1] = pp.mbits[2] = pp.mbits[3] = 0u;
}

__device__ __forceinline__ float c_sin_rev(float thi, float tlo, float scale, int h) {
    const float f = __builtin_amdgcn_fractf(thi * scale);
    return __builtin_amdgcn_sinf(fmaf(tlo, scale, f + (h ? 0.25f : 0.f)));
}

template <int L, int KSN> __device__ __forceinline__ void c_encode(const float (&x)[3], int h, XBlk& out) {
    float thi[3], tlo[3];
#pragma unroll
    for (int c = 0; c < 3; ++c) {
        thi[c] = x[c] * 0.15915494309189535f;
        tlo[c] = fmaf(x[c], 0.15915494309189535f, -thi[c]) + x[c] * 6.4206383e-09f;
    }
    f32x16 r[2];
    unsigned m = 0u;
#pragma unroll
    for (int q = 0; q < 32; q += 2) {
        float y[2];
#pragma unroll
        for (int i = 0; i < 2; ++i) {
            const int qq = q + i;
            if (qq >= KSN * 8) y[i] = 0.f;
            else if (qq < 3 * L) y[i] = c_sin_rev(thi[qq % 3], tlo[qq % 3], (float)(1 << (qq / 3)), h);
            else if (qq == 3 * L) y[i] = h ? x[1] : x[0];
            else if (qq == 3 * L + 1) y[i] = h ? 0.f : x[2];
            else y[i] = 0.f;
        }
        r[0][q >> 1] = y[0];
        r[1][q >> 1] = y[1];
    }
#pragma unroll
    for (int v = 0; v < 16; ++v) c_drain_pair<false>(r[0], r[1], v, out, m);
    c_finish(out, m, r[0], r[1]);
}

}
```

### evdeblurnerf_amd/csrc/nerf_mlp.h

```cpp
#pragma once

#include <cstddef>
#include <cstdint>

namespace evd {

constexpr int PE_L = 10;
constexpr int PE_LV = 4;
constexpr int PE_KS = (3 * PE_L + 2 + 7) / 8;
constexpr int PEV_KS = (3 * PE_LV + 2 + 7) / 8;
constexpr int PE_L_MAX = (8 * PE_KS - 2) / 3;
__host__ __device__ constexpr int pe_ksteps(int L) { return (3 * L + 2 + 7) / 8; }

__host__ __device__ constexpr int phi(int kk) { return 8 * ((kk & 7) >> 2) + 4 * (kk >> 3) + (kk & 3); }
__host__ __device__ constexpr int phi_inv(int p) { return (p & 3) | ((p >> 3) << 2) | (((p >> 2) & 1) << 3); }

__host__ __device__ constexpr int pe_src_col(int L, int q, int h) {
    return q < 3 * L ? 3 + 6 * (q / 3) + 3 * h + (q % 3) : (q == 3 * L ? h : (q == 3 * L + 1 ? (h == 0 ? 2 : -1) : -1));
}

constexpr bool is_half_prec(int prec) { return prec == 2  || prec == 3 ; }
constexpr bool is_train_prec(int prec) { return is_half_prec(prec) || prec == 1 ; }
constexpr int frag_bytes(int prec) { return is_half_prec(prec) ? 1024 : 2048; }
constexpr int mlp_threads(int prec) { return is_half_prec(prec) ? 512 : 256; }
constexpr int chunk_bytes(int prec) { return mlp_threads(prec) * 64; }
constexpr int frags_per_chunk(int prec) { return chunk_bytes(prec) / frag_bytes(prec); }

constexpr int nerf_group(int prec) { return 1; }

struct MlpParams {
    const char* wstream;
    const float* bias;
    const float* ray_batch;
    const float* z;
    long nsamp;
    int S, ncol, D, skip, nchunks, nbias;
    float* raw;
    float* feature;
    int feature_kind;
    char* act;
    int pe_l, pe_lv;
    int no_views;
    const unsigned* wscale;
};

namespace astore {
constexpr int PE = 0, DIR = 4, H0 = 6;
constexpr int F = H0 + 16 * 8, HV = F + 16, FWD_END = HV + 8;
constexpr int G_RGB = FWD_END, G_ALPHA = G_RGB + 1;
constexpr int D_HV = G_ALPHA + 1, D_F = D_HV + 8, D_H0 = D_F + 16;
constexpr int D_PE0 = D_H0 + 16 * 8, D_PE5 = D_PE0 + PE_KS, D_DIRG = D_PE5 + PE_KS;
constexpr int M_H0 = D_DIRG + PEV_KS, M_HV = M_H0 + 8;
constexpr int TILE_FRAGS = M_HV + 1;
constexpr long TILE_BYTES = (long)TILE_FRAGS * 1024;
constexpr long tile_bytes(int prec) { return (long)TILE_FRAGS * frag_bytes(prec); }
}

}
```

### evdeblurnerf_amd/csrc/nerf_mlp_c_kernel.h

```cpp
#pragma once

#include "mlp_pipe_c.h"

namespace evd {

template <int W, int D, int SKIP, bool TRAIN = false> struct NerfNetC {
    static constexpr int T = W / 32, KB = W / 64;
    static constexpr bool FOLD = !TRAIN;
    static constexpr int slot(int s) { return TRAIN ? s : -1; }
    static constexpr int oslot(int l) { return slot(astore::H0 + 16 * l); }
    static constexpr int pslot(int l) { return slot(astore::H0 + 16 * l + 4 * (KB - 1)); }
    static constexpr int mslot(int l) { return slot(astore::M_H0 + l); }
    static_assert(!TRAIN || (W == 256 && D == 8), "the activation store is laid out for the 8 x 256 network");
    static_assert(PE_KS == 4 && PEV_KS == 2 && T % 2 == 0 && KB >= 2, "block structure of the encodings and the hidden width");
    static constexpr bool is_wide(int l) { return l - 1 == SKIP; }
    typedef CLayer<1, 4, T, 2, true, false, 0, 0, 0, false, 0, 2, oslot(0), -1, mslot(0)> L0;
    static constexpr int CH_HID = CLayer<KB, 4, T, 2, true, false, 0, 0, 2, true, KB - 1, 2>::NCHUNKS;
    static constexpr int CH_WIDE = CLayer<KB + 1, 4, T, 2, true, false, 0, 0, 2, true, KB, 2>::NCHUNKS;
    static constexpr int chunk0(int l) {
        int c = L0::NCHUNKS;
        for (int i = 1; i < l; ++i) c += is_wide(i) ? CH_WIDE : CH_HID;
        return c;
    }
    static constexpr int PARH = L0::PAR_OUT;
    static_assert((T / 2) % 2 == 0, "accumulator parity");
    template <int l> using Hidden = std::conditional_t<is_wide(l),
        CLayer<KB + 1, 4, T, 2, true, false, chunk0(l), PARH, 2, true, KB, l == D - 1 ? 1 : 2, oslot(l), pslot(l - 1), mslot(l), mslot(l - 1), 4 * (KB - 1)>,
        CLayer<KB, 4, T, 2, true, false, chunk0(l), PARH, 2, true, KB - 1, l == D - 1 ? 1 : 2, oslot(l), pslot(l - 1), mslot(l), mslot(l - 1)>>;
    typedef CLayer<KB, 4, 1, 1, false, true, chunk0(D), PARH, 2, true, KB - 1, 2, -1, pslot(D - 1), -1, mslot(D - 1)> Alpha;
    typedef CLayer<KB, 4, T, 2, false, false, Alpha::CHUNK0 + Alpha::NCHUNKS, Alpha::PAR_OUT, 0, false, 0, 2, slot(astore::F)> Feature;
    typedef std::conditional_t<FOLD,
        CLayer<KB + 1, 2, T / 2, 2, true, false, Alpha::CHUNK0 + Alpha::NCHUNKS, Alpha::PAR_OUT, 0, false, 0, 1>,
        CLayer<KB + 1, 2, T / 2, 2, true, false, Feature::CHUNK0 + Feature::NCHUNKS, Feature::PAR_OUT, 2, false, KB - 1, 1, slot(astore::HV),
               slot(astore::F + 4 * (KB - 1)), slot(astore::M_HV)>> Views;
    typedef CLayer<KB / 2, 4, 1, 1, false, true, Views::CHUNK0 + Views::NCHUNKS, Views::PAR_OUT, 2, true, KB / 2 - 1, 0, -1, slot(astore::HV + 4 * (KB / 2 - 1)), -1,
                   slot(astore::M_HV)> Rgb;
    static constexpr int NCH = Rgb::CHUNK0 + Rgb::NCHUNKS;
    static constexpr int NTILES = D * T + 1 + (FOLD ? 0 : T) + T / 2 + 1;
    static_assert(D >= 2 && NTILES * 32 <= CCfg::BIAS_WORDS / 2, "bias / row-scale block");
};

template <class N, class ST> struct NerfCtxC {
    ST st;
    CPipe pp;
    XBlk buf[2][N::KB];
    XBlk pe, pev;
    lds_f32_p bias;
    int lane;
    CAct act;
};

template <class N, class ST, int l, int D, bool TRAIN = false> struct HiddenLoopC {
    static __device__ __forceinline__ void run(NerfCtxC<N, ST>& cx) {
        typedef typename N::template Hidden<l> L;
        constexpr int KB = N::KB, T = N::T;
        lds_f32_p lb = cx.bias + l * T * 32;
        if constexpr (l + 1 < D) {
            typedef typename N::template Hidden<l + 1> NX;
            step<L, NX>(cx, lb);
            HiddenLoopC<N, ST, l + 1, D, TRAIN>::run(cx);
        } else {
            step<L, typename N::Alpha>(cx, lb);
        }
    }
    template <class L, class NX> static __device__ __forceinline__ void step(NerfCtxC<N, ST>& cx, lds_f32_p lb) {
        constexpr int KB = N::KB;
        if constexpr (N::is_wide(l)) {
            XBlk wide[KB + 1];
#pragma unroll
            for (int j = 0; j < KB - 1; ++j) wide[j] = cx.buf[(l - 1) & 1][j];
            wide[KB - 1] = cx.pe;
            c_layer<L, NX, ST, KB + 1, KB, TRAIN>(cx.st, cx.pp, wide, cx.buf[l & 1], nullptr, lb, cx.lane, cx.act);
        } else {
            c_layer<L, NX, ST, KB, KB, TRAIN>(cx.st, cx.pp, cx.buf[(l - 1) & 1], cx.buf[l & 1], nullptr, lb, cx.lane, cx.act);
        }
    }
};

template <int W, int D, int SKIP, bool TRAIN = false>
__global__ __launch_bounds__(CCfg::NT, 1) void k_nerf_mlp_c(const MlpParams p) {
    typedef NerfNetC<W, D, SKIP, TRAIN> N;
    typedef CStream<N::NCH> ST;
    constexpr int T = N::T, KB = N::KB;
    extern __shared__ __attribute__((aligned(16))) char smem[];

    pipe_fp16_saturate<EVD_PREC_F16>();
    const int tid = threadIdx.x, lane = tid & 63, wave = tid >> 6;
    const int n = lane & 31, h = lane >> 5;
    ST st0;
    st0.start_issue(p.wstream, smem, tid);
    float* bias = reinterpret_cast<float*>(smem + CCfg::RING);
    {
        constexpr int NB = (CCfg::BIAS_WORDS / 2 / 4 + CCfg::NT - 1) / CCfg::NT;
        f32x4 bv[NB];
        u32x4 sv[NB];
#pragma unroll
        for (int q = 0; q < NB; ++q) {
            const int i = (tid + q * CCfg::NT) * 4;
            bv[q] = i < p.nbias ? *reinterpret_cast<const f32x4*>(p.bias + i) : f32x4{0.f, 0.f, 0.f, 0.f};
            sv[q] = i < p.nbias ? *reinterpret_cast<const u32x4*>(p.wscale + i) : u32x4{0u, 0u, 0u, 0u};
        }
#pragma unroll
        for (int q = 0; q < NB; ++q) {
            const int i = (tid + q * CCfg::NT) * 4;
            if (i < p.nbias) {
                *reinterpret_cast<f32x4*>(bias + i) = bv[q];
                *reinterpret_cast<u32x4*>(reinterpret_cast<unsigned*>(bias) + CCfg::BIAS_WORDS / 2 + i) = sv[q];
            }
        }
    }
    unsigned bias_off = lds_offset_of(bias);
    asm volatile("" : "+v"(bias_off));
    const lds_f32_p lbias = (lds_f32_p)(unsigned long)bias_off;

    const long ntile = TRAIN ? (p.nsamp + 255) / 256 * (256 / CCfg::SAMPLES) : (p.nsamp + CCfg::SAMPLES - 1) / CCfg::SAMPLES;
    for (long tile = blockIdx.x;;) {
    NerfCtxC<N, ST> cx;
    cx.st = st0;
    cx.bias = lbias;
    cx.lane = lane;
    const long smp = tile * CCfg::SAMPLES + wave * 32 + n;
    const bool valid = smp < p.nsamp;
    const long sidx = valid ? smp : p.nsamp - 1;
    {
        const long ray = sidx / p.S;
        const float* rb = p.ray_batch + ray * p.ncol;
        const float zv = p.z[sidx];
        float pts[3], vd[3];
#pragma unroll
        for (int c = 0; c < 3; ++c) {
            pts[c] = __fadd_rn(rb[c], __fmul_rn(rb[3 + c], zv));
            vd[c] = rb[8 + c];
        }
        c_encode<PE_L, PE_KS>(pts, h, cx.pe);
        c_encode<PE_LV, PEV_KS>(vd, h, cx.pev);
    }
    cx.act = CAct{};
    if constexpr (TRAIN) {
        const long t32 = __builtin_amdgcn_readfirstlane((int)(tile * (CCfg::SAMPLES / 32) + wave));
        cx.act.base = p.act + t32 * astore::TILE_BYTES;
        cx.act.voff = lane * 16;
        c_store_input<PE_KS>(cx.act, astore::PE, cx.pe);
        c_store_input<PEV_KS>(cx.act, astore::DIR, cx.pev);
    }

    cx.st.start_wait();
    c_prime<typename N::L0>(cx.st, cx.pp, lbias, lane);
    {
        XBlk in_pe[1];
        in_pe[0] = cx.pe;
        c_layer<typename N::L0, typename N::template Hidden<1>, ST, 1, KB, TRAIN>(cx.st, cx.pp, in_pe, cx.buf[0], nullptr, lbias, lane, cx.act);
    }
    HiddenLoopC<N, ST, 1, D, TRAIN>::run(cx);

    XBlk (&hact)[KB] = cx.buf[(D - 1) & 1];
    lds_f32_p lb = lbias + D * T * 32;
    float araw[4], rraw[4];
    XBlk none[1];
    typedef std::conditional_t<N::FOLD, typename N::Views, typename N::Feature> AfterAlpha;
    c_layer<typename N::Alpha, AfterAlpha, ST, KB, 1, TRAIN>(cx.st, cx.pp, hact, none, araw, lb, lane, cx.act);
    lb += 32;
    XBlk hbuf[KB / 2];
    if constexpr (N::FOLD) {
        XBlk hv[KB + 1];
#pragma unroll
        for (int j = 0; j < KB; ++j) hv[j] = hact[j];
        hv[KB] = cx.pev;
        c_layer<typename N::Views, typename N::Rgb, ST, KB + 1, KB / 2, TRAIN>(cx.st, cx.pp, hv, hbuf, nullptr, lb, lane, cx.act);
    } else {
        XBlk vin[KB + 1];
        c_layer<typename N::Feature, typename N::Views, ST, KB, KB + 1, TRAIN>(cx.st, cx.pp, hact, vin, nullptr, lb, lane, cx.act);
        lb += T * 32;
        vin[KB] = cx.pev;
        c_layer<typename N::Views, typename N::Rgb, ST, KB + 1, KB / 2, TRAIN>(cx.st, cx.pp, vin, hbuf, nullptr, lb, lane, cx.act);
    }
    lb += (T / 2) * 32;
    c_layer<typename N::Rgb, void, ST, KB / 2, 1, TRAIN>(cx.st, cx.pp, hbuf, none, rraw, lb, lane, cx.act);
    const bool more = tile + gridDim.x < ntile;
    if (more) cx.st.restart_issue();

    if (h == 0 && valid) {
        f32x4 o = {rraw[0], rraw[1], rraw[2], araw[0]};
        *reinterpret_cast<f32x4*>(p.raw + sidx * 4) = o;
    }
    if (!more) break;
    tile += gridDim.x;
    }
}

template <int W, int D, int SKIP, bool TRAIN = false> constexpr int nerf_c_chunks() { return NerfNetC<W, D, SKIP, TRAIN>::NCH; }

template <int W, int D, int SKIP, bool TRAIN = false>
static int launch_nerf_c(const MlpParams& p, hipStream_t st) {
    typedef NerfNetC<W, D, SKIP, TRAIN> N;
    const long tiles = TRAIN ? cdiv(p.nsamp, 256L) * (256 / CCfg::SAMPLES) : cdiv(p.nsamp, CCfg::SAMPLES);
    const long blocks = cmin_l(tiles, (long)c_persistent_blocks());
    const size_t lds = CCfg::TOTAL;
    EVD_SET_MAX_LDS((&k_nerf_mlp_c<W, D, SKIP, TRAIN>), lds);
    if (TRAIN != (p.act != nullptr)) return fail(EVD_E_INVALID, "evd_nerf_mlp (f16c): the activation store goes with the training launch");
    if (p.nbias != N::NTILES * 32) return fail(EVD_E_INVALID, "evd_nerf_mlp (f16c): %d bias floats, kernel expects %d", p.nbias, N::NTILES * 32);
    if (p.nchunks != N::NCH) return fail(EVD_E_INVALID, "evd_nerf_mlp (f16c): packed stream has %d chunks, kernel expects %d", p.nchunks, N::NCH);
    if (!p.wscale) return fail(EVD_E_INVALID, "evd_nerf_mlp (f16c): no row scales");
    hipLaunchKernelGGL((k_nerf_mlp_c<W, D, SKIP, TRAIN>), dim3((unsigned)blocks), dim3(CCfg::NT), lds, st, p);
    EVD_LAUNCH_CHECK();
    return EVD_OK;
}

constexpr bool nerf_c_built(int W, int D, int skip) { return W == 256 && D == 8 && skip == 4; }


}
```

### evdeblurnerf_amd/csrc/nerf_net.h

```cpp
#pragma once

#include "evd_common.h"
#include "pack.h"

enum { EVD_BWD_RGB = 0, EVD_BWD_VIEWS, EVD_BWD_HEAD, EVD_BWD_PE0, EVD_BWD_PESKIP, EVD_BWD_DIR, EVD_BWD_HIDDEN1, EVD_BWD_NSTREAMS = EVD_BWD_HIDDEN1 + EVD_MAX_LAYERS };

struct evd_nerf {
    typedef evd::PackedStream Packed;
    int D, W, skip, rgb_act, sigma_act;
    int multires = 10, multires_views = 4;
    int no_views = 0;
    float rmnear;
    Packed stream[EVD_NUM_PREC];
    int nchunks[EVD_NUM_PREC];
    Packed pipe[EVD_NUM_PREC];
    int pipe_chunks[EVD_NUM_PREC];
    evd::DevBuf bias, bias_src;
    evd::PackedStreamC pipe_c;
    evd::PackedStreamC pipe_cf;
    evd::DevBuf bias_f, bias_f_src, fold_arena;
    int fold_chunks = 0;
    Packed bwd[EVD_NUM_PREC][EVD_BWD_NSTREAMS];
    evd::DevBuf wmaps;
    int nparam_blocks;
    long param_off[2 * EVD_MAX_LAYERS + 9];
    evd::RepackBatch batch;
    mutable evd::SideStream side;
};
```

### evdeblurnerf_amd/nerf.py

```python
from __future__ import annotations

import ctypes as C

import numpy as np
import torch

from . import _lib as L


def _np32(v):
    if isinstance(v, torch.Tensor):
        v = v.detach().cpu().numpy()
    return np.ascontiguousarray(v, dtype=np.float32)


class _Raw2Outputs(torch.autograd.Function):

    @staticmethod
    def forward(ctx, raw, z, rd, noise, sigma_ch, rgb_ch0, rgb_act, sigma_act, white_bkgd, thr):
        R, S, Cc = raw.shape
        dev = raw.device
        rgb = torch.empty((R, 3), dtype=torch.float32, device=dev)
        dens = torch.empty((R, S - 1), dtype=torch.float32, device=dev)
        acc = torch.empty((R,), dtype=torch.float32, device=dev)
        wts = torch.empty((R, S), dtype=torch.float32, device=dev)
        depth = torch.empty((R,), dtype=torch.float32, device=dev)
        L.check(L.lib().evd_raw2outputs(L.ptr(raw), L.ptr(z), L.ptr(rd), rd.shape[-1], R, S, Cc, sigma_ch, rgb_ch0, 3, rgb_act, sigma_act,
                                        int(bool(white_bkgd)), thr, L.ptr(noise), L.ptr(rgb), L.ptr(dens), L.ptr(acc), L.ptr(wts),
                                        L.ptr(depth), None, 0, None, L.stream_ptr()), "evd_raw2outputs")
        ctx.save_for_backward(raw, z, rd, noise if noise is not None else torch.empty(0, device=dev))
        ctx.cfg = (sigma_ch, rgb_ch0, rgb_act, sigma_act, int(bool(white_bkgd)), thr, noise is not None)
        ctx.mark_non_differentiable(dens)
        ctx.set_materialize_grads(False)
        return rgb, dens, acc, wts, depth

    @staticmethod
    def backward(ctx, g_rgb, g_dens, g_acc, g_wts, g_depth):
        raw, z, rd, noise = ctx.saved_tensors
        sigma_ch, rgb_ch0, rgb_act, sigma_act, white, thr, has_noise = ctx.cfg
        R, S, Cc = raw.shape
        c = lambda g: g.contiguous().float() if g is not None else None
        d_raw = torch.empty_like(raw)
        d_rd = torch.empty_like(rd) if ctx.needs_input_grad[2] else None
        L.check(L.lib().evd_raw2outputs_bwd_rays(L.ptr(raw), L.ptr(z), L.ptr(rd), rd.shape[-1], R, S, Cc, sigma_ch, rgb_ch0, 3, rgb_act, sigma_act,
                                                 white, thr, L.ptr(noise) if has_noise else None, L.ptr(c(g_rgb)), L.ptr(c(g_depth)),
                                                 L.ptr(c(g_acc)), L.ptr(c(g_wts)), L.ptr(d_raw), L.ptr(d_rd), rd.shape[-1], L.stream_ptr()),
                "evd_raw2outputs_bwd_rays")
        return (d_raw, None, d_rd) + (None,) * 7


class _NerfMLP(torch.autograd.Function):

    @staticmethod
    def forward(ctx, flat, ray_batch, z_vals, net, precision):
        raw, store = net.mlpforward_train(ray_batch, z_vals, precision)
        ctx.net, ctx.precision, ctx.store = net, precision, store
        ctx.rb, ctx.z = ray_batch, z_vals
        ctx.accum = getattr(flat, "_evd_accum", None)
        return raw

    @staticmethod
    def backward(ctx, d_raw):
        L.note_backward()
        d_rb = None
        acc = ctx.accum() if (ctx.accum is not None and ctx.needs_input_grad[0] and not torch.is_grad_enabled()) else None
        if ctx.needs_input_grad[1]:
            rb, z = ctx.rb.detach().contiguous().float(), ctx.z.detach().contiguous().float()
            pts = (rb[:, None, 0:3] + rb[:, None, 3:6] * z[..., None]).contiguous()
            g, d_pts, d_dirs = ctx.net.mlp_backward_flat(d_raw, ctx.store, ctx.precision, pts=pts, ray_batch=rb, accumulate_into=acc)
            d_rb = torch.zeros_like(rb)
            d_pts = d_pts.reshape(pts.shape)
            d_rb[:, 0:3] = d_pts.sum(1)
            d_rb[:, 3:6] = (d_pts * z[..., None]).sum(1)
            d_rb[:, 8:11] = d_dirs.reshape(pts.shape).sum(1)
        else:
            g = ctx.net.mlp_backward_flat(d_raw, ctx.store, ctx.precision, accumulate_into=acc)
        ctx.store = None
        return g, d_rb, None, None, None


class NeRF:

    def __init__(self, state_dict, prefix="", D=8, W=256, multires=10, multires_views=4, skips=(4,),
                 rgb_activate="sigmoid", sigma_activate="relu", render_rmnearplane=0,
                 extract_feature="after_linear", composite_feature=True, precision="f16x3", use_viewdirs=True):
        self.D, self.W = D, W
        self.use_viewdirs = bool(use_viewdirs)
        self.multires, self.multires_views = multires, multires_views
        self.rgb_activate, self.sigma_activate = rgb_activate, sigma_activate
        self.render_rmnearplane = render_rmnearplane
        self.extract_feature, self.composite_feature = extract_feature, composite_feature
        self.precision = precision
        self.training = False
        g = lambda k: _np32(state_dict[prefix + k]) if (prefix + k) in state_dict else None
        keep = []
        d = L.NerfDesc()
        d.D, d.W, d.multires, d.multires_views = D, W, multires, multires_views
        d.skip = skips[0] if len(skips) else -1
        d.rgb_act, d.sigma_act, d.rmnear = L.ACT[rgb_activate], L.ACT[sigma_activate], float(render_rmnearplane)
        fp = lambda a: a.ctypes.data_as(C.POINTER(C.c_float)) if a is not None else None
        for i in range(D):
            w, b = g(f"pts_linears.{i}.weight"), g(f"pts_linears.{i}.bias")
            if w is None or b is None:
                raise L.EvdError(f"state dict lacks {prefix}pts_linears.{i}")
            keep += [w, b]
            d.pts_w[i], d.pts_b[i] = fp(w), fp(b)
        if self.use_viewdirs:
            for name, key in (("views", "views_linears.0"), ("feature", "feature_linear"), ("alpha", "alpha_linear"),
                              ("rgb", "rgb_linear")):
                w, b = g(key + ".weight"), g(key + ".bias")
                keep += [w, b]
                setattr(d, name + "_w", fp(w))
                setattr(d, name + "_b", fp(b))
        else:
            w, b = g("output_linear.weight"), g("output_linear.bias")
            if w is None or b is None:
                raise L.EvdError(f"state dict lacks {prefix}output_linear (use_viewdirs=False)")
            keep += [w, b]
            d.output_w, d.output_b, d.output_ch = fp(w), fp(b), int(w.shape[0])
        h = C.c_void_p()
        L.check(L.lib().evd_nerf_create(C.byref(d), C.byref(h)), "evd_nerf_create")
        self._h = h

    def __del__(self):
        h = getattr(self, "_h", None)
        if h and L is not None and getattr(L, "lib", None) is not None:
            L.lib().evd_nerf_destroy(h)
            self._h = None

    @property
    def handle(self):
        return self._h

    def train(self, mode=True):
        self.training = mode
        return self

    def stream_bytes(self, precision=None):
        return int(L.lib().evd_nerf_stream_bytes(self._h, L.PREC[precision or self.precision]))

    def mlpforward(self, ray_batch, z_vals, want_feature=False, precision=None):
        rb = ray_batch.contiguous().float()
        z = z_vals.contiguous().float()
        ncol = 11 if self.use_viewdirs else 8
        if rb.shape[1] != ncol:
            raise L.EvdError(f"mlpforward needs the {ncol}-column ray batch (use_viewdirs={self.use_viewdirs})")
        if want_feature and not self.use_viewdirs and self.extract_feature == "after_linear":
            raise L.EvdError('a use_viewdirs=False network has no "after_linear" feature (nerf.py:159)')
        R, S = z.shape
        raw = torch.empty((R, S, 4), dtype=torch.float32, device=z.device)
        feat = torch.empty((R, S, self.W), dtype=torch.float32, device=z.device) if want_feature else None
        kind = 2 if self.extract_feature == "before_linear" else 1
        L.check(L.lib().evd_nerf_mlp(self._h, L.PREC[precision or self.precision], L.ptr(rb), L.ptr(z), R, S,
                                     L.ptr(raw), L.ptr(feat), kind, L.stream_ptr()), "evd_nerf_mlp")
        return raw, feat

    def mlpforward_train(self, ray_batch, z_vals, precision=None):
        if not self.use_viewdirs:
            raise L.EvdError("the training path is not built for use_viewdirs=False networks")
        rb = ray_batch.contiguous().float()
        z = z_vals.contiguous().float()
        R, S = z.shape
        raw = torch.empty((R, S, 4), dtype=torch.float32, device=z.device)
        nb = int(L.lib().evd_nerf_train_store_bytes_prec(L.PREC[precision or self.precision], R * S))
        if nb == 0 and R * S > 0:
            raise L.EvdError(f"the training path is built for precision f16 / bf16 / f16x3 / f16c / f16m, not {precision or self.precision}")
        store = torch.empty((nb,), dtype=torch.uint8, device=z.device)
        L.check(L.lib().evd_nerf_mlp_train(self._h, L.PREC[precision or self.precision], L.ptr(rb), L.ptr(z), R, S, L.ptr(raw),
                                            L.ptr(store), nb, L.stream_ptr()), "evd_nerf_mlp_train")
        return raw, store

    def param_blocks(self):
        if getattr(self, "_blocks", None) is None:
            nb = 2 * self.D + 8
            off = (C.c_long * (nb + 1))()
            if L.lib().evd_nerf_param_blocks(self._h, off, nb + 1) != nb:
                raise L.EvdError("evd_nerf_param_blocks: unexpected parameter block count")
            W, D = self.W, self.D
            keys = [(f"pts_linears.{l}", W, None) for l in range(D)] + [("views_linears.0", W // 2, None), ("feature_linear", W, None),
                                                                       ("alpha_linear", 1, None), ("rgb_linear", 3, None)]
            blocks = []
            for i, (k, o, _) in enumerate(keys):
                nw = off[2 * i + 1] - off[2 * i]
                blocks.append((k + ".weight", (o, nw // o), off[2 * i]))
                blocks.append((k + ".bias", (o,), off[2 * i + 1]))
            self._blocks, self._nparam = blocks, off[nb]
        return self._blocks

    def flat_params(self, state_dict, prefix="", device="cuda"):
        blocks = self.param_blocks()
        flat = torch.zeros((self._nparam,), dtype=torch.float32)
        for key, shape, off in blocks:
            if prefix + key in state_dict:
                flat[off:off + int(np.prod(shape))] = torch.as_tensor(_np32(state_dict[prefix + key])).reshape(-1)
        return flat.to(device).requires_grad_(True)

    def unflatten(self, flat):
        return {key: flat[off:off + int(np.prod(shape))].view(shape) for key, shape, off in self.param_blocks()}

    def load_params(self, flat):
        f = flat.detach().contiguous().float()
        self.param_blocks()
        if f.numel() != self._nparam:
            raise L.EvdError(f"flat parameter tensor has {f.numel()} elements, the network {self._nparam}")
        L.check(L.lib().evd_nerf_load_params(self._h, L.ptr(f), L.stream_ptr()), "evd_nerf_load_params")
        self._synced = (flat.data_ptr(), flat._version, L.backward_generation())

    def mlp_train(self, flat, ray_batch, z_vals, precision=None):
        if getattr(self, "_synced", None) != (flat.data_ptr(), flat._version, L.backward_generation()):
            self.load_params(flat)
        return _NerfMLP.apply(flat, ray_batch, z_vals, self, precision or self.precision)

    def mlp_backward_flat(self, d_raw, store, precision=None, pts=None, ray_batch=None, accumulate_into=None):
        g = d_raw.contiguous().float()
        R, S = g.shape[:2]
        blocks = self.param_blocks()
        flat = accumulate_into if accumulate_into is not None else torch.zeros((self._nparam,), dtype=torch.float32, device=g.device)
        gs = L.NerfGrads()
        gs.accumulate = int(accumulate_into is not None)
        base = flat.data_ptr()
        for key, shape, off in blocks:
            name, kind = key.rsplit(".", 1)
            field = "_w" if kind == "weight" else "_b"
            if name.startswith("pts_linears."):
                getattr(gs, "pts" + field)[int(name.split(".")[1])] = base + 4 * off
            else:
                head = {"views_linears.0": "views", "feature_linear": "feature", "alpha_linear": "alpha", "rgb_linear": "rgb"}[name]
                setattr(gs, head + field, base + 4 * off)
        nb = int(L.lib().evd_nerf_backward_workspace_bytes())
        ws = torch.empty((nb,), dtype=torch.uint8, device=g.device)
        want = pts is not None
        d_pts = torch.empty((R * S, 3), dtype=torch.float32, device=g.device) if want else None
        d_dirs = torch.empty((R * S, 3), dtype=torch.float32, device=g.device) if want else None
        vd = ray_batch[:, 8:11] if want else None
        L.check(L.lib().evd_nerf_mlp_backward(self._h, L.PREC[precision or self.precision], L.ptr(g), R, S, L.ptr(store), store.numel(),
                                               C.byref(gs), L.ptr(pts), C.c_void_p(vd.data_ptr()) if want else None, 11, L.ptr(d_pts), L.ptr(d_dirs),
                                               L.ptr(ws), nb, L.stream_ptr()), "evd_nerf_mlp_backward")
        if accumulate_into is not None:
            flat = None
        return (flat, d_pts, d_dirs) if want else flat

    def mlp_backward(self, d_raw, store, precision=None):
        return self.unflatten(self.mlp_backward_flat(d_raw, store, precision))

    def raw2outputs(self, raw, z_vals, rays_d, feature=None, raw_noise_std=0, white_bkgd=False, pytest=False,
                    noise=None):
        raw = raw.contiguous().float()
        z = z_vals.contiguous().float()
        rd = rays_d.contiguous().float()
        R, S, Cc = raw.shape
        dev = raw.device
        if raw_noise_std > 0. and noise is None:
            noise = torch.randn((R, S - 1), dtype=torch.float32, device=dev) * raw_noise_std
        rgb = torch.empty((R, 3), dtype=torch.float32, device=dev)
        dens = torch.empty((R, S - 1), dtype=torch.float32, device=dev)
        acc = torch.empty((R,), dtype=torch.float32, device=dev)
        wts = torch.empty((R, S), dtype=torch.float32, device=dev)
        depth = torch.empty((R,), dtype=torch.float32, device=dev)
        F = feature.shape[-1] if feature is not None else 0
        fmap = torch.empty((R, F), dtype=torch.float32, device=dev) if feature is not None else None
        ft = feature.contiguous().float() if feature is not None else None
        thr = float(self.render_rmnearplane) / 128.0 if (not self.training and self.render_rmnearplane > 0) else 0.0
        nz = noise.contiguous().float() if noise is not None else None
        if raw.requires_grad and torch.is_grad_enabled() and feature is None and Cc == 4:
            rgb, dens, acc, wts, depth = _Raw2Outputs.apply(raw, z, rd, nz, 3, 0, L.ACT[self.rgb_activate], L.ACT[self.sigma_activate],
                                                            white_bkgd, thr)
            return rgb, dens, acc, wts, depth, None
        L.check(L.lib().evd_raw2outputs(L.ptr(raw), L.ptr(z), L.ptr(rd), rd.shape[-1], R, S, Cc, 3, 0, 3,
                                        L.ACT[self.rgb_activate], L.ACT[self.sigma_activate], int(bool(white_bkgd)),
                                        thr, L.ptr(nz), L.ptr(rgb), L.ptr(dens), L.ptr(acc), L.ptr(wts), L.ptr(depth),
                                        L.ptr(ft), F, L.ptr(fmap), L.stream_ptr()), "evd_raw2outputs")
        return rgb, dens, acc, wts, depth, fmap

    def forward(self, ray_batch, z_vals, raw_noise_std=0., white_bkgd=False, is_train=False, want_feature=False):
        raw, feature = self.mlpforward(ray_batch, z_vals, want_feature=want_feature)
        rays_d = ray_batch[:, 3:6]
        if self.composite_feature:
            rgb, _, acc, wts, depth, fmap = self.raw2outputs(raw, z_vals, rays_d, feature, raw_noise_std, white_bkgd)
        else:
            rgb, _, acc, wts, depth, _ = self.raw2outputs(raw, z_vals, rays_d, None, raw_noise_std, white_bkgd)
            fmap = feature
        return rgb, depth, acc, wts, fmap

    __call__ = forward
```

### include/evdnerf.h

```cpp
#ifndef EVDNERF_H
#define EVDNERF_H

#include <stddef.h>

#ifdef __cplusplus
extern "C" {
#endif

#define EVD_OK 0
#define EVD_E_INVALID (-1)
#define EVD_E_HIP (-2)
#define EVD_E_WORKSPACE (-3)
#define EVD_E_NODEVICE (-4)

#define EVD_MAX_LAYERS 16

#define EVD_PREC_F32 0
#define EVD_PREC_F16X3 1
#define EVD_PREC_BF16 2
#define EVD_PREC_F16 3
#define EVD_PREC_F16C 4
#define EVD_NUM_PREC 5
#define EVD_PREC_F16M 5

#define EVD_ACT_NONE 0
#define EVD_ACT_RELU 1
#define EVD_ACT_SIGMOID 2
#define EVD_ACT_EXP 3
#define EVD_ACT_SIGMOID1 4
#define EVD_ACT_SOFTPLUS 5
#define EVD_ACT_TANH 6

const char* evd_last_error(void);
int evd_version(void);
long evd_debug_side_spin_count(void);
int evd_device_count(void);

int evd_get_rays(int H, int W, const float* K, const float* c2w, int add_halfpix, float* rays_o, float* rays_d, void* stream);
int evd_get_rays_pix(const float* coords, const float* K, const float* c2ws, long n, int add_halfpix,
                     float* rays_o, float* rays_d, void* stream);
int evd_ndc_rays(int H, int W, float focal, float near, const float* rays_o, const float* rays_d, long n,
                 float* out_o, float* out_d, void* stream);
int evd_rbk_warp(const float* rays, const float* r, const float* v, long R, int M, int use_origin, float* new_rays, float* transforms,
                 void* stream);
typedef struct {
    int C, W_r, W_v, W_w, D_r, D_v, D_w, M, use_origin, n_img;
    float rv_window;
} evd_rigid_blur_desc;
typedef struct {
    const float* table;
    const float *r_branch_w, *r_branch_b, *v_branch_w, *v_branch_b, *w_branch_w, *w_branch_b;
    const float *r_linear_w, *r_linear_b, *v_linear_w, *v_linear_b;
    const float *w_linear_w, *w_linear_b;
} evd_rigid_blur_params;
size_t evd_rigid_blur_workspace_bytes(const evd_rigid_blur_desc* d, long R);
int evd_rigid_blur_forward(const evd_rigid_blur_desc* d, const evd_rigid_blur_params* p, const float* rays, const long* ids, const float* x, long R,
                           float* new_rays, float* weight, float* img_embed, void* stream);
int evd_rigid_blur_backward(const evd_rigid_blur_desc* d, const evd_rigid_blur_params* p, const float* rays, const long* ids, const float* x, long R,
                            const float* d_new_rays, const float* d_weight, const float* d_img_embed, float* grads, float* d_rays, float* d_x,
                            void* workspace, size_t workspace_bytes, void* stream);
int evd_numerics_flags(const float* const* ptrs, const long* counts, int n_keys, unsigned* flags, void* stream);
int evd_embed(const float* x, long n, int dim, int L, float* out, void* stream);

typedef struct {
    int H, W;
    float focal;
    int ndc, use_viewdirs, lindisp, N_samples, N_importance, white_bkgd;
    float near, far, perturb;
    int is_train;
    int precision;
} evd_render_cfg;

int evd_ray_batch(const evd_render_cfg* cfg, const float* rays, long R, float* ray_batch, void* stream);
int evd_ray_batch_bwd(const evd_render_cfg* cfg, const float* rays, const float* d_ray_batch, long R, float* d_rays, void* stream);
int evd_points(const float* ray_batch, int ncol, const float* z, long R, int S, float* pts, void* stream);
int evd_points_bwd(const float* z, const float* d_pts, long R, int S, int accumulate, float* d_ray_batch, void* stream);
int evd_sample_z(const evd_render_cfg* cfg, const float* ray_batch, int ncol, long R, const float* t_rand,
                 float* z, void* stream);
int evd_sample_z_pts(const evd_render_cfg* cfg, const float* ray_batch, int ncol, long R, const float* t_rand,
                     float* z, float* pts, void* stream);
int evd_ray_batch_z(const evd_render_cfg* cfg, const float* rays, long R, const float* t_rand, float* ray_batch, float* z,
                    void* stream);

typedef struct evd_nerf evd_nerf;

typedef struct {
    int D, W, multires, multires_views, skip;
    int rgb_act, sigma_act;
    float rmnear;
    const float *pts_w[EVD_MAX_LAYERS], *pts_b[EVD_MAX_LAYERS];
    const float *views_w, *views_b, *feature_w, *feature_b, *alpha_w, *alpha_b, *rgb_w, *rgb_b;
    const float *output_w, *output_b;
    int output_ch;
} evd_nerf_desc;

int evd_nerf_create(const evd_nerf_desc* desc, evd_nerf** out);
void evd_nerf_destroy(evd_nerf* net);
long evd_nerf_param_count(const evd_nerf* net);
int evd_nerf_param_blocks(const evd_nerf* net, long* offsets, int capacity);
int evd_nerf_load_params(evd_nerf* net, const float* params, void* stream);
size_t evd_nerf_stream_bytes(const evd_nerf* net, int precision);

int evd_nerf_mlp(const evd_nerf* net, int precision, const float* ray_batch, const float* z, long R, int S,
                 float* raw, float* feature, int feature_kind, void* stream);

size_t evd_nerf_train_store_bytes(long nsamp);
size_t evd_nerf_train_store_bytes_prec(int precision, long nsamp);
int evd_nerf_mlp_train(const evd_nerf* net, int precision, const float* ray_batch, const float* z, long R, int S,
                       float* raw, void* store, size_t store_bytes, void* stream);

typedef struct {
    float *pts_w[EVD_MAX_LAYERS], *pts_b[EVD_MAX_LAYERS];
    float *views_w, *views_b, *feature_w, *feature_b, *alpha_w, *alpha_b, *rgb_w, *rgb_b;
    int accumulate;
} evd_nerf_grads;

size_t evd_nerf_backward_workspace_bytes(void);
int evd_nerf_mlp_backward(const evd_nerf* net, int precision, const float* d_raw, long R, int S, void* store, size_t store_bytes,
                          const evd_nerf_grads* grads, const float* pts, const float* viewdirs, int vd_stride, float* d_pts,
                          float* d_dirs, void* workspace, size_t workspace_bytes, void* stream);

int evd_raw2outputs(const float* raw, const float* z, const float* rays_d, int rays_d_stride, long R, int S, int C,
                    int sigma_ch, int rgb_ch0, int n_rgb, int rgb_act, int sigma_act, int white_bkgd,
                    float rmnear_thresh, const float* noise,
                    float* out_map, float* density, float* acc, float* weights, float* depth,
                    const float* feature, int F, float* fmap, void* stream);

int evd_raw2outputs_bwd(const float* raw, const float* z, const float* rays_d, int rays_d_stride, long R, int S, int C,
                        int sigma_ch, int rgb_ch0, int n_rgb, int rgb_act, int sigma_act, int white_bkgd, float rmnear_thresh,
                        const float* noise, const float* g_map, const float* g_depth, const float* g_acc, const float* g_weights,
                        float* d_raw, void* stream);
int evd_raw2outputs_bwd_rays(const float* raw, const float* z, const float* rays_d, int rays_d_stride, long R, int S, int C,
                             int sigma_ch, int rgb_ch0, int n_rgb, int rgb_act, int sigma_act, int white_bkgd, float rmnear_thresh,
                             const float* noise, const float* g_map, const float* g_depth, const float* g_acc, const float* g_weights,
                             float* d_raw, float* d_rays_d, int d_rays_d_stride, void* stream);

int evd_sample_pdf_merge(const float* z, const float* weights, long R, int S, int N, int det, const float* u,
                         float* z_samples, float* z_merged, int* order, float* z_std, void* stream);

typedef struct {
    float *rgb, *depth, *acc;
    float *z_vals, *weights;
    float *rgb0, *depth0, *acc0, *z_std;
    float *z_vals0, *weights0;
    float *feature;
    float *raw;
    int feature_kind;
} evd_render_out;

size_t evd_nerf_render_workspace_bytes(const evd_render_cfg* cfg, long R);
int evd_nerf_render_rays(const evd_nerf* coarse, const evd_nerf* fine, const evd_render_cfg* cfg, const float* ray_batch,
                         long R, const float* t_rand, const float* u, const float* noise0, const float* noise1,
                         evd_render_out* out, void* workspace, size_t workspace_bytes, void* stream);
int evd_nerf_render(const evd_nerf* coarse, const evd_nerf* fine, const evd_render_cfg* cfg, const float* rays, long R,
                    const float* t_rand, const float* u, const float* noise0, const float* noise1,
                    evd_render_out* out, void* workspace, size_t workspace_bytes, void* stream);

typedef struct evd_voxel evd_voxel;

typedef struct {
    int num_layers, hidden_dim, geo_feat_dim, num_layers_color, input_ch, multires, multires_views;
    int app_dim, n_comp[3], grid[3], app_act, rgb_act, sigma_act, composite_feature;
    float aabb[6], rmnear;
    const float *sigma_w[EVD_MAX_LAYERS];
    const float *color_w[EVD_MAX_LAYERS], *color_b[EVD_MAX_LAYERS];
    const float *plane[3], *line[3], *basis;
} evd_voxel_desc;

int evd_voxel_create(const evd_voxel_desc* desc, evd_voxel** out);
void evd_voxel_destroy(evd_voxel* v);
int evd_voxel_sample(const evd_voxel* v, const float* pts, long n, float* out, int out_stride, int out_col, void* stream);
int evd_voxel_sample_prec(const evd_voxel* v, int precision, const float* pts, long n, float* out, int out_stride, int out_col, void* stream);
int evd_voxel_forward(const evd_voxel* v, int precision, const float* pts, const float* viewdirs, int vd_stride, const float* fts, int F,
                      const float* z, const float* rays_d, int rays_d_stride, long R, int S, int is_train,
                      float* color, float* depth, float* acc, float* weights, float* feature,
                      void* workspace, size_t workspace_bytes, void* stream);
size_t evd_voxel_forward_workspace_bytes(const evd_voxel* v, long R, int S);
size_t evd_c2f_render_workspace_bytes(const evd_voxel* coarse, const evd_voxel* fine, const evd_render_cfg* cfg, long R);
int evd_c2f_render_rays(const evd_voxel* coarse, const evd_voxel* fine, const evd_render_cfg* cfg, const float* ray_batch, long R,
                        const float* t_rand, const float* u, const float* noise0, const float* noise1,
                        evd_render_out* out, void* workspace, size_t workspace_bytes, void* stream);
int evd_c2f_render(const evd_voxel* coarse, const evd_voxel* fine, const evd_render_cfg* cfg, const float* rays, long R,
                   const float* t_rand, const float* u, const float* noise0, const float* noise1,
                   evd_render_out* out, void* workspace, size_t workspace_bytes, void* stream);
int evd_merge_features(const float* old, const float* fresh, const int* order, long R, int S, int N, int F, float* out, int out_stride, void* stream);
int evd_merge_features_bwd(const float* d_out, int d_stride, const int* order, long R, int S, int N, int F, float* d_old, float* d_fresh, void* stream);
int evd_voxel_tv_loss(const evd_voxel* v, float* out, void* stream);

typedef struct { float *sigma_w[2], *color_w[3], *color_b[3]; int accumulate;  } evd_voxel_grads;
int evd_voxel_geo_feat_dim(const evd_voxel* v);
long evd_voxel_param_count(const evd_voxel* v);
int evd_voxel_param_blocks(const evd_voxel* v, long* offsets, int capacity);
int evd_voxel_load_params(evd_voxel* v, const float* params, void* stream);
size_t evd_voxel_train_store_bytes(const evd_voxel* v, long nsamp);
size_t evd_voxel_train_store_bytes_prec(const evd_voxel* v, int precision, long nsamp);
size_t evd_voxel_backward_workspace_bytes(void);
int evd_voxel_mlp_train(const evd_voxel* v, int precision, const float* pts, const float* viewdirs, int vd_stride, const float* fts,
                        int ft_stride, long R, int S, float* raw, float* feature, void* store, size_t store_bytes, void* stream);
int evd_voxel_mlp_backward(const evd_voxel* v, int precision, const float* d_raw, const float* raw, const float* d_feature,
                           const void* awp_store, size_t awp_store_bytes, long R, int S, void* store, size_t store_bytes, const evd_voxel_grads* grads, float* d_fts, int d_fts_stride, const float* pts,
                           const float* viewdirs, int vd_stride, float* d_pts, float* d_dirs, void* workspace,
                           size_t workspace_bytes, void* stream);

typedef struct { float *plane[3], *line[3], *basis; } evd_voxel_grid_grads;
int evd_voxel_grid_sizes(const evd_voxel* v, long* sizes);
int evd_voxel_get_grids(const evd_voxel* v, float* const* plane, float* const* line, float* basis, void* stream);
int evd_voxel_load_grids(evd_voxel* v, const float* const* plane, const float* const* line, const float* basis, void* stream);
int evd_voxel_sample_bwd(const evd_voxel* v, const float* pts, long n, const float* d_out, int d_stride, int d_col,
                         const evd_voxel_grid_grads* g, float* d_pts, void* stream);
size_t evd_voxel_sample_bwd_workspace_bytes(const evd_voxel* v, long n);
int evd_voxel_sample_bwd_ws(const evd_voxel* v, const float* pts, long n, const float* d_out, int d_stride, int d_col,
                            const evd_voxel_grid_grads* g, float* d_pts, void* workspace, size_t workspace_bytes, void* stream);
int evd_voxel_sample_bwd_prec(const evd_voxel* v, int precision, const float* pts, long n, const float* d_out, int d_stride, int d_col,
                              const evd_voxel_grid_grads* g, float* d_pts, void* workspace, size_t workspace_bytes, void* stream);
int evd_voxel_tv_loss_bwd(const evd_voxel* v, const float* d_loss, const evd_voxel_grid_grads* g, void* stream);

int evd_weighted_sum(const float* x, const float* ccw, long R, int P, int C, float* out, void* stream);

typedef struct evd_crf evd_crf;
typedef struct {
    int map_type;
    float gamma;
    int extra_features;
    const float *w[4], *b[4];
} evd_crf_desc;
int evd_crf_create(const evd_crf_desc* desc, evd_crf** out);
void evd_crf_destroy(evd_crf* crf);
int evd_crf_forward(const evd_crf* crf, const float* x, const float* feat, int feat_per_channel, int skip_learn,
                    int luma, long n, float* out, void* stream);

int evd_blur_loss_reduce(const evd_crf* crf_rgb, int skip_learn, const float* rgb_p, const float* rgb0_p,
                         const float* w1, const float* w2, const float* tgt, const float* tgt0, long R, int P,
                         float* partial, float* out_rgb, float* out_rgb1, float* out_awp, void* stream);

int evd_blur_loss_bwd(const evd_crf* crf_rgb, int skip_learn, const float* rgb_p, const float* rgb0_p, const float* w1, const float* w2,
                      const float* tgt, const float* tgt0, long R, int P, const float* g_partial, float* d_rgb_p, float* d_rgb0_p,
                      float* d_w1, float* d_w2, void* stream);
int evd_blur_loss_bwd_dev(const evd_crf* crf_rgb, int skip_learn, const float* rgb_p, const float* rgb0_p, const float* w1, const float* w2,
                          const float* tgt, const float* tgt0, long R, int P, const float* g_partial_dev, float* d_rgb_p, float* d_rgb0_p,
                          float* d_w1, float* d_w2, void* stream);

int evd_event_loss_reduce(const evd_crf* crf_ev, int skip_learn, int add_bii_feat, int tonemap_only,
                          const float* start, const float* end, const float* start0, const float* end0,
                          const float* cum_neg, const float* cum_pos, float thr_neg, float thr_pos,
                          const unsigned char* color_mask, const float* color_weight, long N,
                          float* partial, void* stream);

int evd_crf_param_count(void);
int evd_crf_get_params(const evd_crf* crf, float* host_params);
int evd_crf_load_params(evd_crf* crf, const float* host_params);
int evd_event_loss_bwd(const evd_crf* crf_ev, int skip_learn, int add_bii_feat, int tonemap_only,
                       const float* start, const float* end, const float* start0, const float* end0,
                       const float* cum_neg, const float* cum_pos, float thr_neg, float thr_pos,
                       const unsigned char* color_mask, const float* color_weight, long N, float g_fine, float g_coarse,
                       float* d_start, float* d_end, float* d_start0, float* d_end0, float* d_params, void* stream);
int evd_event_loss_bwd_dev(const evd_crf* crf_ev, int skip_learn, int add_bii_feat, int tonemap_only,
                           const float* start, const float* end, const float* start0, const float* end0,
                           const float* cum_neg, const float* cum_pos, float thr_neg, float thr_pos,
                           const unsigned char* color_mask, const float* color_weight, long N, const float* g_partial_dev,
                           float* d_start, float* d_end, float* d_start0, float* d_end0, float* d_params, void* stream);

int evd_awp_feature_integration(const float* feat, const float* z, const float* rays_d, long N, int S, int C, float* out, void* stream);
int evd_awp_feature_integration_bwd(const float* feat, const float* z, const float* rays_d, const float* d_out, long N, int S, int C,
                                    float* d_feat, float* d_z, float* d_rays_d, void* stream);

int evd_mam_local_forward(const float* h_local, const float* u, long R, int P, int S, int C, float* h_inter, float* h_intra, float* alpha,
                          float* beta, void* stream);
int evd_mam_local_backward(const float* h_local, const float* u, const float* alpha, const float* beta, const float* h_inter,
                           const float* h_intra, const float* d_inter, const float* d_intra, long R, int P, int S, int C, float* d_h_local,
                           float* d_u_partial, int accumulate, unsigned* d_h_absmax, void* stream);

typedef struct {
    int P, S, VF, dir_freqs, n_mot, training;
    float bn_eps, bn_momentum;
} evd_awp_tail_desc;
int evd_awp_tail_num_params(int n_mot);
long evd_awp_tail_param_count(const evd_awp_tail_desc* d);
size_t evd_awp_tail_workspace_bytes(const evd_awp_tail_desc* d, long R, int backward);
long evd_awp_tail_saved_floats(const evd_awp_tail_desc* d);
int evd_awp_tail_forward(const evd_awp_tail_desc* d, const float* const* params, const float* h, const float* view_feature,
                         const float* rays_d, const float* h_inter, const float* h_intra, long R, float* bn_running_mean,
                         float* bn_running_var, long long* bn_num_batches, float* out, float* saved_y, float* saved_xg, float* saved_stats,
                         float* saved_rays, void* workspace, size_t workspace_bytes, void* stream);
int evd_awp_tail_backward(const evd_awp_tail_desc* d, const float* const* params, const float* h, const float* view_feature,
                          const float* rays_d, const float* h_inter, const float* h_intra, long R, const float* saved_y,
                          const float* saved_xg, const float* saved_stats, const float* saved_rays, const float* d_out, float* d_h,
                          float* d_view_feature,
                          float* d_rays_d, float* d_h_inter, float* d_h_intra, float* d_params, void* workspace, size_t workspace_bytes,
                          void* stream);

int evd_awp_local_consumers_backward(const float* h_local, const float* u, const float* alpha, const float* beta, const float* h_inter,
                                     const float* h_intra, const float* d_inter, const float* d_intra, const float* z, const float* rays_d,
                                     const float* d_integrated, long R, int P, int S, int C, float* d_h_local, float* d_u_partial, float* d_z,
                                     float* d_rays_d, unsigned* d_h_absmax, void* stream);

typedef struct evd_awp_embed evd_awp_embed;
typedef struct { float *w[4], *b[4]; } evd_awp_embed_grads;
int evd_awp_embed_create(const float* const* weights, const float* const* biases, int input_ch, int width, int depth, evd_awp_embed** out);
void evd_awp_embed_destroy(evd_awp_embed* a);
long evd_awp_embed_param_count(const evd_awp_embed* a);
int evd_awp_embed_load_params(evd_awp_embed* a, const float* params, void* stream);
size_t evd_awp_embed_store_bytes(const evd_awp_embed* a, long nsamp);
size_t evd_awp_embed_backward_workspace_bytes(void);
int evd_awp_embed_forward(const evd_awp_embed* a, int precision, const float* geo_rows, const evd_voxel* fine, const void* fine_store,
                          size_t fine_store_bytes, long nsamp, float* h_local, void* store, size_t store_bytes, void* stream);
int evd_awp_embed_backward(const evd_awp_embed* a, int precision, const float* d_h_local, long nsamp, void* store, size_t store_bytes,
                           const evd_awp_embed_grads* grads, float* d_geo_rows, const unsigned* d_h_absmax, void* workspace,
                           size_t workspace_bytes, void* stream);

int evd_edi_deblur(const float* blurry, const float* bii, int steps, long npix, float* sharp, void* stream);
int evd_edi_bii_image(const float* x, const float* y, const signed char* p, long n, int w, int h,
                      float c_pos, float c_neg, float* image, void* stream);
size_t evd_edi_prior_workspace_bytes(int n_img, int steps, int h, int w);
int evd_edi_prior(const double* events, long N, const double* id_to_coords, long n_coords, const double* boundaries, const float* images,
                  int n_img, int steps, int h, int w, float c_pos, float c_neg, float* prior_out, long long* windows_out, int* bad_id,
                  void* workspace, size_t workspace_bytes, void* stream);

size_t evd_compute_successor_workspace_bytes(long N);
int evd_compute_successor(const int* pixel_ids, long N, long HW, long long* successor, int* num_successors,
                          long long* latest_seen, long long* first_seen, void* workspace, size_t workspace_bytes, void* stream);

int evd_sample_events(const double* events, long N, int ncol, const float* id_to_coords, long n_coords, const unsigned char* id_to_color_map,
                      const float* poses, const long long* events_ids, const long long* hops, long n, const float* K, int add_halfpix,
                      float* rays_start, float* rays_end, float* pos_cumsum, float* neg_cumsum, long long* coords_ids,
                      unsigned char* color_map, long long* successor, int* mismatch, void* stream);

typedef struct evd_pose_track {
    int n_keys;
    const double* key_t;
    const double* key_quat;
    const double* key_rotvec;
    const double* trans_coef;
    float bd_scale;
    int recenter;
    double recenter_inv[12];
} evd_pose_track;
int evd_interpolate_poses(const evd_pose_track* track, const double* t, long n, float* poses, void* stream);
int evd_sample_events_track(const double* events, long N, int ncol, const float* id_to_coords, long n_coords, const unsigned char* id_to_color_map,
                            const evd_pose_track* track, const long long* events_ids, const long long* hops, long n, const float* K,
                            int add_halfpix, float* rays_start, float* rays_end, float* pos_cumsum, float* neg_cumsum, long long* coords_ids,
                            unsigned char* color_map, long long* successor, int* mismatch, void* stream);

size_t evd_event_coord_ids_workspace_bytes(long N, int h, int w);
int evd_event_coord_ids(const float* x, const float* y, long N, int h, int w, long long* ev_coord_ids, long long* noev_coord_ids, double* id_to_coords,
                        long long* counts, void* workspace, size_t workspace_bytes, void* stream);
size_t evd_event_filter_workspace_bytes(long N);
int evd_event_filter(const long long* coord_ids, const double* t, const double* p, long N, double tmin, double tmax, double* events_out, long long* count,
                     int* bad_polarity, void* workspace, size_t workspace_bytes, void* stream);
size_t evd_event_color_map_workspace_bytes(long n_coords);
int evd_event_color_map(const double* id_to_coords, long n_coords, int h, int w, const float* inv_mapx, const float* inv_mapy, const long long* noev_coord_ids,
                        long n_noev, unsigned char* id_to_color_map, int* unmapped, void* workspace, size_t workspace_bytes, void* stream);

int evd_image_batch(const long long* ray_ids, long n, const float* images, const float* pts0_images, const float* poses, int n_img, int H,
                    int W, const float* K, float* rays, float* rays_x, float* rays_y, long long* images_idx, float* rgbsf, float* poses_out,
                    float* rgbsf_pts0, int* invalid, void* stream);

#define EVD_IMG_METRICS_TILE_H 16
#define EVD_IMG_METRICS_TILE_W 32
size_t evd_img_metrics_workspace_bytes(int B, int H, int W);
int evd_img_metrics(const float* pred, const float* target, const float* mask, int mask_ch, int B, int H, int W, int margin_h, int margin_w,
                    double* out, void* workspace, size_t workspace_bytes, void* stream);
int evd_to8b(const float* x, long n, unsigned char* out, void* stream);

#define EVD_LPIPS_MIN_SIDE 31
#define EVD_LPIPS_LAYERS 5
typedef struct evd_lpips_model evd_lpips_model;
typedef struct {
    const float *conv_w[EVD_LPIPS_LAYERS], *conv_b[EVD_LPIPS_LAYERS];
    const float* lin[EVD_LPIPS_LAYERS];
    float shift[3], scale[3];
} evd_lpips_desc;
int evd_lpips_create(const evd_lpips_desc* desc, evd_lpips_model** out);
void evd_lpips_destroy(evd_lpips_model* m);
size_t evd_lpips_workspace_bytes(int B, int H, int W);
int evd_lpips(const evd_lpips_model* m, const float* pred, const float* target, int B, int H, int W, double* out, void* workspace, size_t workspace_bytes,
              void* stream);

int evd_probe_mfma_rate(int random_operands, int iters, double* tflops, void* stream);

#ifdef __cplusplus
}
#endif
#endif
```

Baseline: 5.571 million rays/s.

## Compute view-direction term once per ray in f32 instead of per-sample MFMA

Adds a RAYVIEW variant of the folded f16c inference kernel. The view-direction encoding block is dropped from the packed weight stream, and its 128x27 contribution is computed in f32 per lane from LDS-resident weights. The result is stored as a per-wave bias vector that seeds the accumulators of the views layer. This removes the MFMAs and weight chunks for the direction columns, relying on the view direction being constant across each 32-sample wave when S is a multiple of 32. In exchange it adds LDS use (100 KiB), a per-wave scalar dot-product loop, extra packing state and a debug launch counter.

```diff
diff --git a/evdeblurnerf_amd/_lib.py b/evdeblurnerf_amd/_lib.py
--- a/evdeblurnerf_amd/_lib.py
+++ b/evdeblurnerf_amd/_lib.py
@@ -157,6 +157,7 @@
     "evd_nerf_param_blocks": (_I, [_vp, C.POINTER(C.c_long), _I]),
     "evd_nerf_load_params": (_I, [_vp, _vp, _vp]),
     "evd_nerf_stream_bytes": (_S, [_vp, _I]),
+    "evd_nerf_debug_rayview_launches": (_L, [_vp]),
     "evd_nerf_mlp": (_I, [_vp, _I, _vp, _vp, _L, _I, _vp, _vp, _I, _vp]),
     "evd_nerf_train_store_bytes": (_S, [_L]),
     "evd_nerf_train_store_bytes_prec": (_S, [_I, _L]),
diff --git a/evdeblurnerf_amd/csrc/evd_api.hip b/evdeblurnerf_amd/csrc/evd_api.hip
--- a/evdeblurnerf_amd/csrc/evd_api.hip
+++ b/evdeblurnerf_amd/csrc/evd_api.hip
@@ -31,6 +31,8 @@
 int nerf_mlp_pipe_dispatch(int prec, const MlpParams& p, hipStream_t st);
 int nerf_mlp_c_dispatch(int W, int D, int skip, const MlpParams& p, hipStream_t st);
 int nerf_mlp_c_chunks(int W, int D, int skip, bool train);
+int nerf_mlp_c_rayview_chunks(int W, int D, int skip);
+bool nerf_mlp_c_rayview(int S);
 
 static __global__ void k_fold_feature(const float* __restrict__ views_w, const float* __restrict__ views_b, const float* __restrict__ feature_w,
                                       const float* __restrict__ feature_b, int W, int ICV, float* __restrict__ wfold, float* __restrict__ bfold) {
@@ -60,10 +62,16 @@
                        ext + n->param_off[2 * D + 2], ext + n->param_off[2 * D + 3], W, ICV, ext + total, ext + total + nw);
     EVD_LAUNCH_CHECK();
     int rc = repack_stream_c(n->pipe_cf, ext, st);
+    if (!rc) rc = repack_stream_c(n->pipe_cr, ext, st);
     if (rc) return rc;
     const long nb = (long)(n->bias_f.bytes / sizeof(float));
     hipLaunchKernelGGL(k_gather_f32, dim3((unsigned)cdiv(nb, 256L)), dim3(256), 0, st, (const float*)ext, (const int*)n->bias_f_src.p, nb, (float*)n->bias_f.p);
     EVD_LAUNCH_CHECK();
+    if (n->wdir.p) {
+        const long nd = (long)(n->wdir.bytes / sizeof(float));
+        hipLaunchKernelGGL(k_gather_f32, dim3((unsigned)cdiv(nd, 256L)), dim3(256), 0, st, (const float*)ext, (const int*)n->wdir_src.p, nd, (float*)n->wdir.p);
+        EVD_LAUNCH_CHECK();
+    }
     return EVD_OK;
 }
 
@@ -197,7 +205,7 @@
         if (prec == EVD_PREC_F16C) {
             n->nchunks[prec] = n->pipe_chunks[prec] = 0;
             if (no_views || !standard || !nerf_mlp_c_chunks(W, D, d->skip, false)) continue;
-            auto build_c = [&](StreamBuilderC& sc, const float* base, bool fold) {
+            auto build_c = [&](StreamBuilderC& sc, const float* base, bool fold, bool dirblk) {
                 auto Pb = [&](int i) { return base + n->param_off[i]; };
                 sc.arena = base;
                 const int KB = KS / 4;
@@ -216,7 +224,7 @@
                 }
                 sc.layer(Pb(2 * D + 4), 1, W, 1, KS, 1, c_hid_col);
                 if (!fold) sc.layer(Pb(2 * D + 2), W, W, T, KS, 2, c_hid_col);
-                sc.layer(fold ? base + total : Pb(2 * D), W / 2, W + ICV, T / 2, KS + PEV_KS, 2, [&](int j, int kk) {
+                sc.layer(fold ? base + total : Pb(2 * D), W / 2, W + ICV, T / 2, KS + (dirblk ? PEV_KS : 0), 2, [&](int j, int kk) {
                     if (j < KS) return c_hid_col(j, kk);
                     const int c = pe_src_col(Lv, 8 * (j - KS) + (kk & 7), kk >> 3);
                     return c < 0 ? -1 : W + c;
@@ -224,7 +232,7 @@
                 sc.layer(Pb(2 * D + 6), 3, W / 2, 1, KS / 2, 1, c_hid_col);
             };
             StreamBuilderC sc(PIPE_CB);
-            build_c(sc, A, false);
+            build_c(sc, A, false, true);
             n->pipe_chunks[prec] = (int)(sc.bytes.size() / PIPE_CB);
             if (n->pipe_chunks[prec] != nerf_mlp_c_chunks(W, D, d->skip, true)) rc = fail(EVD_E_INVALID, "evd_nerf_create: f16c stream has %d chunks, kernel expects %d", n->pipe_chunks[prec], nerf_mlp_c_chunks(W, D, d->skip, true));
             if (!rc) rc = n->pipe_c.upload(sc);
@@ -232,11 +240,22 @@
             const long nfold = (long)(W / 2) * (W + ICV) + W / 2;
             std::vector<float> ext((size_t)(total + nfold), 0.f);
             StreamBuilderC sf(PIPE_CB);
-            build_c(sf, ext.data(), true);
+            build_c(sf, ext.data(), true, true);
             n->fold_chunks = (int)(sf.bytes.size() / PIPE_CB);
             if (n->fold_chunks != nerf_mlp_c_chunks(W, D, d->skip, false)) rc = fail(EVD_E_INVALID, "evd_nerf_create: folded f16c stream has %d chunks, kernel expects %d", n->fold_chunks, nerf_mlp_c_chunks(W, D, d->skip, false));
             if (!rc) rc = n->pipe_cf.upload(sf);
             if (!rc) rc = n->fold_arena.alloc(ext.size() * sizeof(float));
+            if (rc) continue;
+            StreamBuilderC sr(PIPE_CB);
+            build_c(sr, ext.data(), true, false);
+            n->ray_chunks = (int)(sr.bytes.size() / PIPE_CB);
+            if (n->ray_chunks != nerf_mlp_c_rayview_chunks(W, D, d->skip)) rc = fail(EVD_E_INVALID, "evd_nerf_create: f16c stream without the direction block has %d chunks, kernel expects %d", n->ray_chunks, nerf_mlp_c_rayview_chunks(W, D, d->skip));
+            if (!rc) rc = n->pipe_cr.upload(sr);
+            std::vector<int32_t> dsrc((size_t)(W / 2) * 28, -1);
+            for (int r = 0; r < W / 2; ++r)
+                for (int j = 0; j < ICV && j < 28; ++j) dsrc[(size_t)r * 28 + j] = (int32_t)(total + (long)r * (W + ICV) + W + j);
+            if (!rc) rc = n->wdir_src.upload(dsrc.data(), dsrc.size() * sizeof(int32_t));
+            if (!rc) rc = n->wdir.alloc(dsrc.size() * sizeof(float));
             continue;
         }
         StreamBuilder sb(prec);
@@ -348,6 +367,9 @@
     n->bias_f.release();
     n->bias_f_src.release();
     n->fold_arena.release();
+    n->pipe_cr.release();
+    n->wdir.release();
+    n->wdir_src.release();
     n->side.release();
     delete n;
 }
@@ -384,6 +406,8 @@
     if (precision == EVD_PREC_F16C) return net->pipe_cf.data.bytes;
     return net->pipe_chunks[precision] ? net->pipe[precision].data.bytes : net->stream[precision].data.bytes;
 }
+
+long evd_nerf_debug_rayview_launches(const evd_nerf* net) { return net ? net->rayview_launches.load(std::memory_order_relaxed) : 0; }
 
 int evd_nerf_mlp(const evd_nerf* net, int precision, const float* ray_batch, const float* z, long R, int S,
                  float* raw, float* feature, int feature_kind, void* stream) {
@@ -410,6 +434,13 @@
         p.wscale = (const unsigned*)net->pipe_cf.scales.p;
         p.bias = (const float*)net->bias_f.p;
         p.nbias = (int)(net->bias_f.bytes / sizeof(float));
+        if (nerf_mlp_c_rayview(S) && net->pipe_cr.data.p && net->wdir.p) {
+            p.wstream = (const char*)net->pipe_cr.data.p;
+            p.nchunks = net->ray_chunks;
+            p.wscale = (const unsigned*)net->pipe_cr.scales.p;
+            p.wdir = (const float*)net->wdir.p;
+            net->rayview_launches.fetch_add(1, std::memory_order_relaxed);
+        }
         return nerf_mlp_c_dispatch(net->W, net->D, net->skip, p, as_stream(stream));
     }
     if (piped) return nerf_mlp_pipe_dispatch(precision, p, as_stream(stream));
diff --git a/evdeblurnerf_amd/csrc/kernel_nerf_mlp_pipe_f16c.hip b/evdeblurnerf_amd/csrc/kernel_nerf_mlp_pipe_f16c.hip
--- a/evdeblurnerf_amd/csrc/kernel_nerf_mlp_pipe_f16c.hip
+++ b/evdeblurnerf_amd/csrc/kernel_nerf_mlp_pipe_f16c.hip
@@ -1,14 +1,23 @@
 #include "nerf_mlp_c_kernel.h"
 
 namespace evd {
+
+typedef NerfNetC<256, 8, 4, false, false> NetFold;
+typedef NerfNetC<256, 8, 4, false, true> NetRay;
+static_assert(NetFold::MFMA16 == 1056 && NetFold::MFMA6 == 532 && NetFold::NCH == 118, "folded inference network: 1588 MFMAs, 118 chunks");
+static_assert(NetRay::MFMA16 == 1048 && NetRay::MFMA6 == 524 && NetRay::NCH == 116, "per-ray view term: 1572 MFMAs, 116 chunks");
+static_assert(NetRay::NTILES == NetFold::NTILES && NetRay::LDS_BYTES == 100 * 1024, "same bias block; 100 KiB of LDS");
 
 int nerf_mlp_c_chunks(int W, int D, int skip, bool train) {
     if (!nerf_c_built(W, D, skip)) return 0;
     return train ? nerf_c_chunks<256, 8, 4, true>() : nerf_c_chunks<256, 8, 4, false>();
 }
+int nerf_mlp_c_rayview_chunks(int W, int D, int skip) { return nerf_c_built(W, D, skip) ? nerf_c_chunks<256, 8, 4, false, true>() : 0; }
+
+bool nerf_mlp_c_rayview(int S) { return S % 32 == 0; }
 
 int nerf_mlp_c_dispatch(int W, int D, int skip, const MlpParams& p, hipStream_t st) {
-    if (nerf_c_built(W, D, skip)) return launch_nerf_c<256, 8, 4>(p, st);
+    if (nerf_c_built(W, D, skip)) return nerf_mlp_c_rayview(p.S) && p.wdir ? launch_nerf_c<256, 8, 4, false, true>(p, st) : launch_nerf_c<256, 8, 4>(p, st);
     return fail(EVD_E_INVALID, "evd_nerf_mlp: EVD_PREC_F16C is built for netdepth 8, netwidth 256, skips [4] only");
 }
 
diff --git a/evdeblurnerf_amd/csrc/mlp_pipe_c.h b/evdeblurnerf_amd/csrc/mlp_pipe_c.h
--- a/evdeblurnerf_amd/csrc/mlp_pipe_c.h
+++ b/evdeblurnerf_amd/csrc/mlp_pipe_c.h
@@ -259,8 +259,9 @@
 
 template <class L> __device__ __forceinline__ constexpr int c_ring_off(int u) { return ((L::CHUNK0 + u / CCfg::UPC) & (CCfg::NSLOT - 1)) * CCfg::CB + (u % CCfg::UPC) * 1024; }
 
-template <class L, class NXT, class ST, int NIN, int NOUT, int P, bool TRAIN = false>
-__device__ __forceinline__ void c_group(ST& st, CPipe& pp, XBlk (&in)[NIN], XBlk (&out)[NOUT], lds_f32_p bias, int lane, const CAct& act = CAct{}) {
+template <class L, class NXT, class ST, int NIN, int NOUT, int P, bool TRAIN = false, int VB = 0>
+__device__ __forceinline__ void c_group(ST& st, CPipe& pp, XBlk (&in)[NIN], XBlk (&out)[NOUT], lds_f32_p bias, int lane, const CAct& act = CAct{},
+                                        lds_f32_p vbias = nullptr) {
     constexpr int G = L::G, NS = L::GROUP_SLOTS;
     constexpr int cur = (L::PAR + P) & 1, oth = cur ^ 1;
     constexpr bool FIRST = P == 0, LAST = P == L::NG - 1;
@@ -279,6 +280,7 @@
     auto bias_thru = [](int s) constexpr { return (NBL == 0 || s <= b0) ? 0 : (s >= NS ? NBL : cmin(NBL, (s - b0) * brate)); };
     const int h = lane >> 5;
     lds_f32_p bias_next = bias + (LAST ? L::TILES : (P + 1) * G) * 32;
+    lds_f32_p bval_next = (LAST ? (VB & 1) != 0 : (VB & 2) != 0) ? vbias + (LAST ? 0 : (P + 1) * G) * 32 : bias_next;
     constexpr int SC_OFF = CCfg::BIAS_WORDS / 2;
     constexpr int ubase = P * L::GROUP_UNITS;
     constexpr int mbase = P * L::KSTEPS * G;
@@ -319,7 +321,7 @@
             if (b < bias_thru(s)) {
                 const int bt = b / 5, q = b % 5;
                 if (q < 4) {
-                    const f32x4 bv = *(lds_f32x4_p)(bias_next + bt * 32 + 8 * q + 4 * h);
+                    const f32x4 bv = *(lds_f32x4_p)(bval_next + bt * 32 + 8 * q + 4 * h);
 #pragma unroll
                     for (int e = 0; e < 4; ++e) pp.acc[oth][bt][4 * q + e] = bv[e];
                 } else {
@@ -432,7 +434,7 @@
         if (bq < NBL) {
             const int bt = bq / 5, q = bq % 5;
             if (q < 4) {
-                const f32x4 bv = *(lds_f32x4_p)(bias_next + bt * 32 + 8 * q + 4 * h);
+                const f32x4 bv = *(lds_f32x4_p)(bval_next + bt * 32 + 8 * q + 4 * h);
 #pragma unroll
                 for (int e = 0; e < 4; ++e) pp.acc[oth][bt][4 * q + e] = bv[e];
             } else {
@@ -442,17 +444,19 @@
     }
 }
 
-template <class L, class NXT, class ST, int NIN, int NOUT, int P, bool TRAIN = false> struct CGroupLoop {
-    static __device__ __forceinline__ void run(ST& st, CPipe& pp, XBlk (&in)[NIN], XBlk (&out)[NOUT], lds_f32_p bias, int lane, const CAct& act = CAct{}) {
-        c_group<L, NXT, ST, NIN, NOUT, P, TRAIN>(st, pp, in, out, bias, lane, act);
-        if constexpr (P + 1 < L::NG) CGroupLoop<L, NXT, ST, NIN, NOUT, P + 1, TRAIN>::run(st, pp, in, out, bias, lane, act);
-    }
-};
-
-template <class L, class NXT, class ST, int NIN, int NOUT, bool TRAIN = false>
-__device__ __forceinline__ void c_layer(ST& st, CPipe& pp, XBlk (&in)[NIN], XBlk (&out)[NOUT], float* out_f32, lds_f32_p bias, int lane, const CAct& act = CAct{}) {
+template <class L, class NXT, class ST, int NIN, int NOUT, int P, bool TRAIN = false, int VB = 0> struct CGroupLoop {
+    static __device__ __forceinline__ void run(ST& st, CPipe& pp, XBlk (&in)[NIN], XBlk (&out)[NOUT], lds_f32_p bias, int lane, const CAct& act = CAct{},
+                                               lds_f32_p vbias = nullptr) {
+        c_group<L, NXT, ST, NIN, NOUT, P, TRAIN, VB>(st, pp, in, out, bias, lane, act, vbias);
+        if constexpr (P + 1 < L::NG) CGroupLoop<L, NXT, ST, NIN, NOUT, P + 1, TRAIN, VB>::run(st, pp, in, out, bias, lane, act, vbias);
+    }
+};
+
+template <class L, class NXT, class ST, int NIN, int NOUT, bool TRAIN = false, int VB = 0>
+__device__ __forceinline__ void c_layer(ST& st, CPipe& pp, XBlk (&in)[NIN], XBlk (&out)[NOUT], float* out_f32, lds_f32_p bias, int lane, const CAct& act = CAct{},
+                                        lds_f32_p vbias = nullptr) {
     static_assert(NIN >= L::NBLK, "input blocks");
-    CGroupLoop<L, NXT, ST, NIN, NOUT, 0, TRAIN>::run(st, pp, in, out, bias, lane, act);
+    CGroupLoop<L, NXT, ST, NIN, NOUT, 0, TRAIN, VB>::run(st, pp, in, out, bias, lane, act, vbias);
     if (L::UNITS % CCfg::UPC != 0) {
         constexpr int c = L::CHUNK0 + L::UNITS / CCfg::UPC, k0 = cmin(CCfg::PIECES, (L::UNITS % CCfg::UPC + 1) / 3);
         if (c + ST::AHEAD < ST::kChunks) {
diff --git a/evdeblurnerf_amd/csrc/nerf_mlp.h b/evdeblurnerf_amd/csrc/nerf_mlp.h
--- a/evdeblurnerf_amd/csrc/nerf_mlp.h
+++ b/evdeblurnerf_amd/csrc/nerf_mlp.h
@@ -42,6 +42,7 @@
     int pe_l, pe_lv;
     int no_views;
     const unsigned* wscale;
+    const float* wdir;
 };
 
 namespace astore {
diff --git a/evdeblurnerf_amd/csrc/nerf_mlp_c_kernel.h b/evdeblurnerf_amd/csrc/nerf_mlp_c_kernel.h
--- a/evdeblurnerf_amd/csrc/nerf_mlp_c_kernel.h
+++ b/evdeblurnerf_amd/csrc/nerf_mlp_c_kernel.h
@@ -1,12 +1,15 @@
 #pragma once
 
+#include <utility>
+
 #include "mlp_pipe_c.h"
 
 namespace evd {
 
-template <int W, int D, int SKIP, bool TRAIN = false> struct NerfNetC {
+template <int W, int D, int SKIP, bool TRAIN = false, bool RAYVIEW = false> struct NerfNetC {
     static constexpr int T = W / 32, KB = W / 64;
     static constexpr bool FOLD = !TRAIN;
+    static_assert(!RAYVIEW || FOLD, "the per-ray view term belongs to the folded inference network");
     static constexpr int slot(int s) { return TRAIN ? s : -1; }
     static constexpr int oslot(int l) { return slot(astore::H0 + 16 * l); }
     static constexpr int pslot(int l) { return slot(astore::H0 + 16 * l + 4 * (KB - 1)); }
@@ -29,15 +32,27 @@
         CLayer<KB, 4, T, 2, true, false, chunk0(l), PARH, 2, true, KB - 1, l == D - 1 ? 1 : 2, oslot(l), pslot(l - 1), mslot(l), mslot(l - 1)>>;
     typedef CLayer<KB, 4, 1, 1, false, true, chunk0(D), PARH, 2, true, KB - 1, 2, -1, pslot(D - 1), -1, mslot(D - 1)> Alpha;
     typedef CLayer<KB, 4, T, 2, false, false, Alpha::CHUNK0 + Alpha::NCHUNKS, Alpha::PAR_OUT, 0, false, 0, 2, slot(astore::F)> Feature;
-    typedef std::conditional_t<FOLD,
-        CLayer<KB + 1, 2, T / 2, 2, true, false, Alpha::CHUNK0 + Alpha::NCHUNKS, Alpha::PAR_OUT, 0, false, 0, 1>,
-        CLayer<KB + 1, 2, T / 2, 2, true, false, Feature::CHUNK0 + Feature::NCHUNKS, Feature::PAR_OUT, 2, false, KB - 1, 1, slot(astore::HV),
-               slot(astore::F + 4 * (KB - 1)), slot(astore::M_HV)>> Views;
+    typedef std::conditional_t<RAYVIEW,
+        CLayer<KB, 4, T / 2, 2, true, false, Alpha::CHUNK0 + Alpha::NCHUNKS, Alpha::PAR_OUT, 0, false, 0, 1>,
+        std::conditional_t<FOLD,
+            CLayer<KB + 1, 2, T / 2, 2, true, false, Alpha::CHUNK0 + Alpha::NCHUNKS, Alpha::PAR_OUT, 0, false, 0, 1>,
+            CLayer<KB + 1, 2, T / 2, 2, true, false, Feature::CHUNK0 + Feature::NCHUNKS, Feature::PAR_OUT, 2, false, KB - 1, 1, slot(astore::HV),
+                   slot(astore::F + 4 * (KB - 1)), slot(astore::M_HV)>>> Views;
     typedef CLayer<KB / 2, 4, 1, 1, false, true, Views::CHUNK0 + Views::NCHUNKS, Views::PAR_OUT, 2, true, KB / 2 - 1, 0, -1, slot(astore::HV + 4 * (KB / 2 - 1)), -1,
                    slot(astore::M_HV)> Rgb;
     static constexpr int NCH = Rgb::CHUNK0 + Rgb::NCHUNKS;
     static constexpr int NTILES = D * T + 1 + (FOLD ? 0 : T) + T / 2 + 1;
     static_assert(D >= 2 && NTILES * 32 <= CCfg::BIAS_WORDS / 2, "bias / row-scale block");
+    static constexpr int VIEWS_BIAS = (D * T + 1) * 32;
+    template <class L> static constexpr int mf16() { return L::NMAIN; }
+    template <class L> static constexpr int mf6() { return 2 * L::NBLK * L::TILES; }
+    template <int... l> static constexpr int hid16(std::integer_sequence<int, l...>) { return (0 + ... + mf16<Hidden<l + 1>>()); }
+    template <int... l> static constexpr int hid6(std::integer_sequence<int, l...>) { return (0 + ... + mf6<Hidden<l + 1>>()); }
+    static constexpr int MFMA16 = mf16<L0>() + hid16(std::make_integer_sequence<int, D - 1>{}) + mf16<Alpha>() + (FOLD ? 0 : mf16<Feature>()) + mf16<Views>() + mf16<Rgb>();
+    static constexpr int MFMA6 = mf6<L0>() + hid6(std::make_integer_sequence<int, D - 1>{}) + mf6<Alpha>() + (FOLD ? 0 : mf6<Feature>()) + mf6<Views>() + mf6<Rgb>();
+    static constexpr int ICV = 3 * (1 + 2 * PE_LV), VR = W / 2, WD_STRIDE = 28, WD_WORDS = VR * WD_STRIDE;
+    static constexpr int LDS_BYTES = CCfg::TOTAL + (RAYVIEW ? (WD_WORDS + CCfg::NW * VR) * 4 : 0);
+    static_assert(!RAYVIEW || (VR == 128 && ICV <= WD_STRIDE && WD_STRIDE % 4 == 0 && LDS_BYTES <= 160 * 1024), "two rows per lane; LDS");
 };
 
 template <class N, class ST> struct NerfCtxC {
@@ -77,9 +92,9 @@
     }
 };
 
-template <int W, int D, int SKIP, bool TRAIN = false>
+template <int W, int D, int SKIP, bool TRAIN = false, bool RAYVIEW = false>
 __global__ __launch_bounds__(CCfg::NT, 1) void k_nerf_mlp_c(const MlpParams p) {
-    typedef NerfNetC<W, D, SKIP, TRAIN> N;
+    typedef NerfNetC<W, D, SKIP, TRAIN, RAYVIEW> N;
     typedef CStream<N::NCH> ST;
     constexpr int T = N::T, KB = N::KB;
     extern __shared__ __attribute__((aligned(16))) char smem[];
@@ -109,9 +124,26 @@
             }
         }
     }
+    if constexpr (RAYVIEW) {
+        constexpr int NV = N::WD_WORDS / 4, NQ = (NV + CCfg::NT - 1) / CCfg::NT;
+        f32x4 wv[NQ];
+#pragma unroll
+        for (int q = 0; q < NQ; ++q) {
+            const int i = tid + q * CCfg::NT;
+            wv[q] = i < NV ? reinterpret_cast<const f32x4*>(p.wdir)[i] : f32x4{0.f, 0.f, 0.f, 0.f};
+        }
+#pragma unroll
+        for (int q = 0; q < NQ; ++q) {
+            const int i = tid + q * CCfg::NT;
+            if (i < NV) reinterpret_cast<f32x4*>(bias + CCfg::BIAS_WORDS)[i] = wv[q];
+        }
+        __syncthreads();
+    }
     unsigned bias_off = lds_offset_of(bias);
     asm volatile("" : "+v"(bias_off));
     const lds_f32_p lbias = (lds_f32_p)(unsigned long)bias_off;
+    const lds_f32_p lwd = lbias + CCfg::BIAS_WORDS;
+    const lds_f32_p vslot = lwd + N::WD_WORDS + wave * N::VR;
 
     const long ntile = TRAIN ? (p.nsamp + 255) / 256 * (256 / CCfg::SAMPLES) : (p.nsamp + CCfg::SAMPLES - 1) / CCfg::SAMPLES;
     for (long tile = blockIdx.x;;) {
@@ -122,7 +154,48 @@
     const long smp = tile * CCfg::SAMPLES + wave * 32 + n;
     const bool valid = smp < p.nsamp;
     const long sidx = valid ? smp : p.nsamp - 1;
-    {
+    if constexpr (RAYVIEW) {
+        const long smp0 = tile * CCfg::SAMPLES + __builtin_amdgcn_readfirstlane(wave) * 32;
+        const long ray = (smp0 < p.nsamp ? smp0 : p.nsamp - 1) / p.S;
+        const float* rb = p.ray_batch + ray * p.ncol;
+        const float zv = p.z[sidx];
+        float pts[3], vd[3];
+#pragma unroll
+        for (int c = 0; c < 3; ++c) {
+            pts[c] = __fadd_rn(rb[c], __fmul_rn(rb[3 + c], zv));
+            vd[c] = rb[8 + c];
+        }
+        c_encode<PE_L, PE_KS>(pts, h, cx.pe);
+        float e[N::WD_STRIDE], thi[3], tlo[3];
+#pragma unroll
+        for (int c = 0; c < 3; ++c) {
+            thi[c] = vd[c] * 0.15915494309189535f;
+            tlo[c] = fmaf(vd[c], 0.15915494309189535f, -thi[c]) + vd[c] * 6.4206383e-09f;
+            e[c] = vd[c];
+        }
+#pragma unroll
+        for (int k = 0; k < PE_LV; ++k) {
+#pragma unroll
+            for (int c = 0; c < 3; ++c) {
+                e[3 + 6 * k + c] = c_sin_rev(thi[c], tlo[c], (float)(1 << k), 0);
+                e[6 + 6 * k + c] = c_sin_rev(thi[c], tlo[c], (float)(1 << k), 1);
+            }
+        }
+        typedef __attribute__((address_space(3))) float* lds_f32_w;
+#pragma unroll
+        for (int rr = 0; rr < 2; ++rr) {
+            const int r = lane + 64 * rr;
+            float u = lbias[N::VIEWS_BIAS + r];
+#pragma unroll
+            for (int q = 0; q < N::WD_STRIDE / 4; ++q) {
+                const f32x4 wq = *(lds_f32x4_p)(lwd + r * N::WD_STRIDE + 4 * q);
+#pragma unroll
+                for (int i = 0; i < 4; ++i)
+                    if (4 * q + i < N::ICV) u = fmaf(wq[i], e[4 * q + i], u);
+            }
+            ((lds_f32_w)vslot)[r] = u;
+        }
+    } else {
         const long ray = sidx / p.S;
         const float* rb = p.ray_batch + ray * p.ncol;
         const float zv = p.z[sidx];
@@ -158,10 +231,12 @@
     float araw[4], rraw[4];
     XBlk none[1];
     typedef std::conditional_t<N::FOLD, typename N::Views, typename N::Feature> AfterAlpha;
-    c_layer<typename N::Alpha, AfterAlpha, ST, KB, 1, TRAIN>(cx.st, cx.pp, hact, none, araw, lb, lane, cx.act);
+    c_layer<typename N::Alpha, AfterAlpha, ST, KB, 1, TRAIN, RAYVIEW ? 1 : 0>(cx.st, cx.pp, hact, none, araw, lb, lane, cx.act, vslot);
     lb += 32;
     XBlk hbuf[KB / 2];
-    if constexpr (N::FOLD) {
+    if constexpr (RAYVIEW) {
+        c_layer<typename N::Views, typename N::Rgb, ST, KB, KB / 2, TRAIN, 2>(cx.st, cx.pp, hact, hbuf, nullptr, lb, lane, cx.act, vslot);
+    } else if constexpr (N::FOLD) {
         XBlk hv[KB + 1];
 #pragma unroll
         for (int j = 0; j < KB; ++j) hv[j] = hact[j];
@@ -188,20 +263,21 @@
     }
 }
 
-template <int W, int D, int SKIP, bool TRAIN = false> constexpr int nerf_c_chunks() { return NerfNetC<W, D, SKIP, TRAIN>::NCH; }
-
-template <int W, int D, int SKIP, bool TRAIN = false>
+template <int W, int D, int SKIP, bool TRAIN = false, bool RAYVIEW = false> constexpr int nerf_c_chunks() { return NerfNetC<W, D, SKIP, TRAIN, RAYVIEW>::NCH; }
+
+template <int W, int D, int SKIP, bool TRAIN = false, bool RAYVIEW = false>
 static int launch_nerf_c(const MlpParams& p, hipStream_t st) {
-    typedef NerfNetC<W, D, SKIP, TRAIN> N;
+    typedef NerfNetC<W, D, SKIP, TRAIN, RAYVIEW> N;
     const long tiles = TRAIN ? cdiv(p.nsamp, 256L) * (256 / CCfg::SAMPLES) : cdiv(p.nsamp, CCfg::SAMPLES);
     const long blocks = cmin_l(tiles, (long)c_persistent_blocks());
-    const size_t lds = CCfg::TOTAL;
-    EVD_SET_MAX_LDS((&k_nerf_mlp_c<W, D, SKIP, TRAIN>), lds);
+    const size_t lds = N::LDS_BYTES;
+    EVD_SET_MAX_LDS((&k_nerf_mlp_c<W, D, SKIP, TRAIN, RAYVIEW>), lds);
     if (TRAIN != (p.act != nullptr)) return fail(EVD_E_INVALID, "evd_nerf_mlp (f16c): the activation store goes with the training launch");
     if (p.nbias != N::NTILES * 32) return fail(EVD_E_INVALID, "evd_nerf_mlp (f16c): %d bias floats, kernel expects %d", p.nbias, N::NTILES * 32);
     if (p.nchunks != N::NCH) return fail(EVD_E_INVALID, "evd_nerf_mlp (f16c): packed stream has %d chunks, kernel expects %d", p.nchunks, N::NCH);
     if (!p.wscale) return fail(EVD_E_INVALID, "evd_nerf_mlp (f16c): no row scales");
-    hipLaunchKernelGGL((k_nerf_mlp_c<W, D, SKIP, TRAIN>), dim3((unsigned)blocks), dim3(CCfg::NT), lds, st, p);
+    if (RAYVIEW && (!p.wdir || p.S % 32 != 0)) return fail(EVD_E_INVALID, "evd_nerf_mlp (f16c): the per-ray view term needs the direction columns and S %% 32 == 0 (S = %d)", p.S);
+    hipLaunchKernelGGL((k_nerf_mlp_c<W, D, SKIP, TRAIN, RAYVIEW>), dim3((unsigned)blocks), dim3(CCfg::NT), lds, st, p);
     EVD_LAUNCH_CHECK();
     return EVD_OK;
 }
diff --git a/evdeblurnerf_amd/csrc/nerf_net.h b/evdeblurnerf_amd/csrc/nerf_net.h
--- a/evdeblurnerf_amd/csrc/nerf_net.h
+++ b/evdeblurnerf_amd/csrc/nerf_net.h
@@ -1,4 +1,6 @@
 #pragma once
+
+#include <atomic>
 
 #include "evd_common.h"
 #include "pack.h"
@@ -20,6 +22,10 @@
     evd::PackedStreamC pipe_cf;
     evd::DevBuf bias_f, bias_f_src, fold_arena;
     int fold_chunks = 0;
+    evd::PackedStreamC pipe_cr;
+    evd::DevBuf wdir, wdir_src;
+    int ray_chunks = 0;
+    mutable std::atomic<long> rayview_launches{0};
     Packed bwd[EVD_NUM_PREC][EVD_BWD_NSTREAMS];
     evd::DevBuf wmaps;
     int nparam_blocks;
diff --git a/evdeblurnerf_amd/nerf.py b/evdeblurnerf_amd/nerf.py
--- a/evdeblurnerf_amd/nerf.py
+++ b/evdeblurnerf_amd/nerf.py
@@ -139,6 +139,9 @@
     def stream_bytes(self, precision=None):
         return int(L.lib().evd_nerf_stream_bytes(self._h, L.PREC[precision or self.precision]))
 
+    def rayview_launches(self):
+        return int(L.lib().evd_nerf_debug_rayview_launches(self._h))
+
     def mlpforward(self, ray_batch, z_vals, want_feature=False, precision=None):
         rb = ray_batch.contiguous().float()
         z = z_vals.contiguous().float()
diff --git a/include/evdnerf.h b/include/evdnerf.h
--- a/include/evdnerf.h
+++ b/include/evdnerf.h
@@ -100,6 +100,7 @@
 int evd_nerf_param_blocks(const evd_nerf* net, long* offsets, int capacity);
 int evd_nerf_load_params(evd_nerf* net, const float* params, void* stream);
 size_t evd_nerf_stream_bytes(const evd_nerf* net, int precision);
+long evd_nerf_debug_rayview_launches(const evd_nerf* net);
 
 int evd_nerf_mlp(const evd_nerf* net, int precision, const float* ray_batch, const float* z, long R, int S,
                  float* raw, float* feature, int feature_kind, void* stream);
```

Result: no change. 5.579 million rays/s, median of 3 (+0.1%).
